# ubc-vision/quadraturefields

Measured on AMD Instinct MI355X. Metric: rays/sec at 800x800 Lego (mesh-quadrature render: ray/mesh intersection + hash-grid/MLP field + compositing), higher is better.
Workload: dtype f32

## Files before the change

### quadraturefields_amd/csrc/exact.hip

```cpp
#include "qf_common.h"
#include "bvh.h"

#pragma clang fp contract(off)

namespace {

constexpr int kMaxHits = QF_BVH_MAX_HITS;

__device__ __forceinline__ bool mt_hit(const float4 a, const float4 b, const float4 c, const float ox, const float oy,
                                       const float oz, const float dx, const float dy, const float dz, float *t_out)
{
    const float e1x = b.x - a.x, e1y = b.y - a.y, e1z = b.z - a.z;
    const float e2x = c.x - a.x, e2y = c.y - a.y, e2z = c.z - a.z;
    const float px = dy * e2z - dz * e2y;
    const float py = dz * e2x - dx * e2z;
    const float pz = dx * e2y - dy * e2x;
    const float det = (e1x * px + e1y * py) + e1z * pz;
    if (!(det != 0.0f)) return false;
    const float inv = 1.0f / det;
    const float tx = ox - a.x, ty = oy - a.y, tz = oz - a.z;
    const float u = ((tx * px + ty * py) + tz * pz) * inv;
    if (!(u >= 0.0f && u <= 1.0f)) return false;
    const float qx = ty * e1z - tz * e1y;
    const float qy = tz * e1x - tx * e1z;
    const float qz = tx * e1y - ty * e1x;
    const float v = ((dx * qx + dy * qy) + dz * qz) * inv;
    if (!(v >= 0.0f && u + v <= 1.0f)) return false;
    const float t = ((e2x * qx + e2y * qy) + e2z * qz) * inv;
    if (!(t > 0.0f)) return false;
    *t_out = t;
    return true;
}

__device__ __forceinline__ float safe_inv(float d)
{
    const float tiny = 1e-30f;
    if (fabsf(d) < tiny) d = (d < 0.0f || (d == 0.0f && signbit(d))) ? -tiny : tiny;
    return 1.0f / d;
}

__device__ __forceinline__ bool hit_less(float ta, int ia, float tb, int ib) { return ta < tb || (ta == tb && ia < ib); }

typedef float f32x4u __attribute__((ext_vector_type(4), aligned(4)));
typedef int i32x4u __attribute__((ext_vector_type(4), aligned(4)));

__device__ __forceinline__ uint64_t hit_key(float t, int id) { return ((uint64_t)__float_as_uint(t) << 32) | (uint32_t)id; }
__device__ __forceinline__ float key_t(uint64_t k) { return __uint_as_float((uint32_t)(k >> 32)); }
__device__ __forceinline__ int key_id(uint64_t k) { return (int)(uint32_t)k; }

template <bool kTri>
__device__ __forceinline__ void sort_row_32(float *row_t, int32_t *row_i, int cnt)
{
    if (kTri) {
        uint64_t key[32];
#pragma unroll
        for (int k = 0; k < 32; ++k) key[k] = k < cnt ? hit_key(row_t[k], row_i[k]) : ~0ull;
#pragma unroll
        for (int k = 2; k <= 32; k <<= 1) {
#pragma unroll
            for (int i = 0; i < 32; ++i) {
                const int l = i ^ (k - 1);
                if (l > i) { const uint64_t a = key[i], b = key[l]; key[i] = a < b ? a : b; key[l] = a < b ? b : a; }
            }
#pragma unroll
            for (int j = k >> 2; j > 0; j >>= 1) {
#pragma unroll
                for (int i = 0; i < 32; ++i) {
                    const int l = i ^ j;
                    if (l > i) { const uint64_t a = key[i], b = key[l]; key[i] = a < b ? a : b; key[l] = a < b ? b : a; }
                }
            }
        }
#pragma unroll
        for (int k = 0; k < 32; ++k)
            if (k < cnt) { row_t[k] = key_t(key[k]); row_i[k] = key_id(key[k]); }
    } else {
        float key[32];
#pragma unroll
        for (int k = 0; k < 32; ++k) key[k] = k < cnt ? row_t[k] : INFINITY;
#pragma unroll
        for (int k = 2; k <= 32; k <<= 1) {
#pragma unroll
            for (int i = 0; i < 32; ++i) {
                const int l = i ^ (k - 1);
                if (l > i) { const float a = key[i], b = key[l]; key[i] = fminf(a, b); key[l] = fmaxf(a, b); }
            }
#pragma unroll
            for (int j = k >> 2; j > 0; j >>= 1) {
#pragma unroll
                for (int i = 0; i < 32; ++i) {
                    const int l = i ^ j;
                    if (l > i) { const float a = key[i], b = key[l]; key[i] = fminf(a, b); key[l] = fmaxf(a, b); }
                }
            }
        }
#pragma unroll
        for (int k = 0; k < 32; ++k)
            if (k < cnt) row_t[k] = key[k];
    }
}

constexpr int kOctRays = 32;
constexpr int kTravThreads = kOctRays * 8;
constexpr int kDone = (int)0x80000000;
constexpr int kMaxPages = 4096;

#define QF_DPP_QUAD_1032 0xB1
#define QF_DPP_QUAD_2301 0x4E
#define QF_DPP_HALF_MIRROR 0x141

__device__ __forceinline__ unsigned oct_min_u32(unsigned v)
{
    v = min(v, (unsigned)__builtin_amdgcn_update_dpp(0, (int)v, QF_DPP_QUAD_1032, 0xf, 0xf, true));
    v = min(v, (unsigned)__builtin_amdgcn_update_dpp(0, (int)v, QF_DPP_QUAD_2301, 0xf, 0xf, true));
    v = min(v, (unsigned)__builtin_amdgcn_update_dpp(0, (int)v, QF_DPP_HALF_MIRROR, 0xf, 0xf, true));
    return v;
}
__device__ __forceinline__ unsigned oct_max_u32(unsigned v)
{
    v = max(v, (unsigned)__builtin_amdgcn_update_dpp(0, (int)v, QF_DPP_QUAD_1032, 0xf, 0xf, true));
    v = max(v, (unsigned)__builtin_amdgcn_update_dpp(0, (int)v, QF_DPP_QUAD_2301, 0xf, 0xf, true));
    v = max(v, (unsigned)__builtin_amdgcn_update_dpp(0, (int)v, QF_DPP_HALF_MIRROR, 0xf, 0xf, true));
    return v;
}
template <int kCtrl>
__device__ __forceinline__ uint64_t dpp_u64(uint64_t v)
{
    const unsigned lo = (unsigned)__builtin_amdgcn_update_dpp(0, (int)(unsigned)v, kCtrl, 0xf, 0xf, true);
    const unsigned hi = (unsigned)__builtin_amdgcn_update_dpp(0, (int)(unsigned)(v >> 32), kCtrl, 0xf, 0xf, true);
    return ((uint64_t)hi << 32) | lo;
}
__device__ __forceinline__ uint64_t oct_max_u64(uint64_t v)
{
    uint64_t o = dpp_u64<QF_DPP_QUAD_1032>(v); v = o > v ? o : v;
    o = dpp_u64<QF_DPP_QUAD_2301>(v); v = o > v ? o : v;
    o = dpp_u64<QF_DPP_HALF_MIRROR>(v); v = o > v ? o : v;
    return v;
}
__device__ __forceinline__ int oct_bcast(int v, int oct_base, int src)
{
    return __builtin_amdgcn_ds_bpermute((oct_base + src) << 2, v);
}
__device__ __forceinline__ void oct_lds_sync()
{
    __builtin_amdgcn_fence(__ATOMIC_ACQ_REL, "wavefront");
    __builtin_amdgcn_wave_barrier();
}

struct OctList {
    uint64_t *keys;
    int K, j;
    int count;
    uint64_t worst;
    int worst_slot;

    __device__ __forceinline__ void find_worst()
    {
        uint64_t m = 0;
        int slot = 0;
        for (int i = j; i < K; i += 8) {
            const uint64_t k = keys[i];
            if (k >= m) { m = k; slot = i; }
        }
        worst = oct_max_u64(m);
        worst_slot = (int)oct_max_u32(m == worst ? (unsigned)slot : 0u);
    }
};

struct TravArgs {
    const float4 *nodes, *tris;
    const float *rays_o, *rays_d;
    int64_t n_rays;
    int root_is_valid, max_hits, image_width, image_height, tiles_x, n_blocks, blocks_per_xcd, stack_cap;
    int stripe_blocks;
    int list_cap;
    float min_sep;
    int32_t *hit_tri;
    float *hit_t;
    int32_t *hit_count;
    uint64_t *keep_mask;
    int32_t *raw_count;
    int tcol_offset;
    const int32_t *all_flag;
};

extern __shared__ uint64_t trav_lds[];

__device__ __forceinline__ uint64_t oct_keep_mask(const TravArgs &a, int64_t ray, int c, int j, int q, int *kept_out)
{
    const int K = a.max_hits, Kc = a.list_cap;
    uint64_t *keys = trav_lds + (size_t)q * Kc;
    uint64_t *sorted = trav_lds + (size_t)kOctRays * Kc + (size_t)q * Kc;
    for (int e = j; e < c; e += 8) keys[e] = hit_key(a.hit_t[ray * K + e], a.hit_tri[ray * K + e]);
    oct_lds_sync();
    for (int e = j; e < c; e += 8) {
        const uint64_t k = keys[e];
        int rank = 0;
        for (int i = 0; i < c; ++i) rank += keys[i] < k ? 1 : 0;
        sorted[rank] = k;
    }
    oct_lds_sync();
    float last = key_t(sorted[0]);
    int kept = 1;
    uint64_t mask = 1ull;
    for (int i = 1; i < c; ++i) {
        const float t = key_t(sorted[i]);
        if (t > last + a.min_sep) { mask |= 1ull << i; ++kept; last = t; }
    }
    oct_lds_sync();
    *kept_out = kept;
    return mask;
}

template <bool kOrdered>
__device__ __forceinline__ void oct_traverse_ray(const TravArgs &ta, int64_t ray, int j, int q, int oct_base)
{
    const int K = ta.max_hits;
    const int Kc = ta.list_cap;
    const float min_sep = ta.min_sep;
    const float4 *__restrict__ nodes = ta.nodes;
    const float4 *__restrict__ tris = ta.tris;
    const int stack_cap = ta.stack_cap;
    uint64_t *keys = trav_lds + (size_t)q * Kc;
    uint64_t *sorted = trav_lds + (size_t)kOctRays * Kc + (size_t)q * Kc;
    int *stack = reinterpret_cast<int *>(trav_lds + (size_t)kOctRays * Kc * (min_sep > 0.0f ? 2 : 1)) + (size_t)q * stack_cap;
    const float *rays_o = ta.rays_o, *rays_d = ta.rays_d;
    const int root_is_valid = ta.root_is_valid;
    float *hit_t = ta.hit_t;
    int32_t *hit_tri = ta.hit_tri, *hit_count = ta.hit_count;
    uint64_t *keep_mask = ta.keep_mask;
    int32_t *raw_count = ta.raw_count;
    const float ox = rays_o[ray * 3], oy = rays_o[ray * 3 + 1], oz = rays_o[ray * 3 + 2];
    const float dx = rays_d[ray * 3], dy = rays_d[ray * 3 + 1], dz = rays_d[ray * 3 + 2];
    const float ix = safe_inv(dx), iy = safe_inv(dy), iz = safe_inv(dz);
    const float nx = -(ox * ix), ny = -(oy * iy), nz = -(oz * iz);
    float *my_t = hit_t + ray * K;
    int32_t *my_tri = hit_tri + ray * K;

    OctList list;
    list.keys = keys; list.K = Kc; list.j = j;
    int kept = 0;
    float last_t = 0.0f;
    uint64_t lo_key = 0;
    float t_lo = 0.0f, t_accept = 0.0f;

    for (int page = 0; page < kMaxPages; ++page) {
        list.count = 0;
        list.worst = ~0ull;
        list.worst_slot = 0;
        float t_limit = INFINITY;
        int sp = 0;
        int cur = root_is_valid ? 0 : kDone;
        while (cur != kDone) {
            while (cur >= 0) {
                const float4 *np = nodes + (size_t)cur * 16 + j * 2;
                const float4 a = np[0];
                const float4 b = np[1];
                const float ax = __builtin_fmaf(a.x, ix, nx), bx = __builtin_fmaf(a.w, ix, nx);
                const float ay = __builtin_fmaf(a.y, iy, ny), by = __builtin_fmaf(b.x, iy, ny);
                const float az = __builtin_fmaf(a.z, iz, nz), bz = __builtin_fmaf(b.y, iz, nz);
                const float tn = fmaxf(fmaxf(fminf(ax, bx), fminf(ay, by)), fmaxf(fminf(az, bz), 0.0f));
                const float tf = fminf(fminf(fmaxf(ax, bx), fmaxf(ay, by)), fmaxf(az, bz)) * 1.0000005f;
                const int tok = __float_as_int(b.z);
                const bool hit = tok != kDone && !(tn > tf) && !(tn * 0.999999f > t_limit) && !(tf < t_lo);
                const unsigned m8 = (unsigned)(__ballot(hit) >> oct_base) & 0xffu;
                if (m8 == 0) {
                    cur = kDone;
                    if (sp > 0) cur = stack[--sp];
                    continue;
                }
                const int n = __popc(m8);
                int nearest;
                if (kOrdered) {
                    const unsigned key = hit ? ((__float_as_uint(tn) & ~7u) | (unsigned)j) : 0xffffffffu;
                    nearest = (int)(oct_min_u32(key) & 7u);
                } else {
                    nearest = __ffs(m8) - 1;
                }
                if (hit && j != nearest) {
                    const unsigned others = m8 & ~(1u << nearest);
                    stack[sp + __popc(others & ((1u << j) - 1u))] = tok;
                }
                sp += n - 1;
                cur = oct_bcast(tok, oct_base, nearest);
                oct_lds_sync();
            }
            if (cur == kDone) break;
            {
                const int packed = ~cur;
                const int first = packed >> 3, cnt = (packed & 7) + 1;
                bool h = false;
                uint64_t key = 0;
                if (j < cnt) {
                    const float4 a = tris[(size_t)(first + j) * 3 + 0];
                    const float4 b = tris[(size_t)(first + j) * 3 + 1];
                    const float4 c = tris[(size_t)(first + j) * 3 + 2];
                    float t;
                    if (mt_hit(a, b, c, ox, oy, oz, dx, dy, dz, &t)) {
                        key = hit_key(t, __float_as_int(a.w));
                        h = key > lo_key && t > t_accept && key < list.worst;
                    }
                }
                const unsigned m8 = (unsigned)(__ballot(h) >> oct_base) & 0xffu;
                if (m8) {
                    const int n = __popc(m8);
                    if (list.count + n <= Kc) {
                        if (h) keys[list.count + __popc(m8 & ((1u << j) - 1u))] = key;
                        list.count += n;
                        oct_lds_sync();
                        if (list.count == Kc) list.find_worst();
                    } else {
                        for (unsigned mm = m8; mm; mm &= mm - 1u) {
                            const int src = __ffs(mm) - 1;
                            const uint64_t k = ((uint64_t)(unsigned)oct_bcast((int)(unsigned)(key >> 32), oct_base, src) << 32) |
                                               (unsigned)oct_bcast((int)(unsigned)key, oct_base, src);
                            if (list.count < Kc) {
                                if (j == 0) keys[list.count] = k;
                                ++list.count;
                                oct_lds_sync();
                                if (list.count == Kc) list.find_worst();
                            } else if (k < list.worst) {
                                if (j == 0) keys[list.worst_slot] = k;
                                oct_lds_sync();
                                list.find_worst();
                            }
                        }
                    }
                    if (list.count == Kc) t_limit = key_t(list.worst);
                }
            }
            cur = kDone;
            if (sp > 0) cur = stack[--sp];
        }

        const int count = list.count;
        if (!(min_sep > 0.0f)) {
            for (int e = j; e < count; e += 8) {
                const uint64_t k = keys[e];
                int rank = 0;
                for (int i = 0; i < count; ++i) rank += keys[i] < k ? 1 : 0;
                my_t[rank] = key_t(k);
                my_tri[rank] = key_id(k);
            }
            kept = count;
            break;
        }
        for (int e = j; e < count; e += 8) {
            const uint64_t k = keys[e];
            int rank = 0;
            for (int i = 0; i < count; ++i) rank += keys[i] < k ? 1 : 0;
            sorted[rank] = k;
        }
        oct_lds_sync();
        for (int i = 0; i < count && kept < K; ++i) {
            const uint64_t k = sorted[i];
            const float t = key_t(k);
            if (kept == 0 || t > last_t + min_sep) {
                if (j == 0) { my_t[kept] = t; my_tri[kept] = key_id(k); }
                ++kept;
                last_t = t;
            }
        }
        if (count < Kc || kept >= K) break;
        lo_key = sorted[Kc - 1];
        t_lo = key_t(lo_key) * 0.999999f;
        t_accept = last_t + min_sep;
        oct_lds_sync();
    }
    for (int i = kept + j; i < K; i += 8) { my_t[i] = INFINITY; my_tri[i] = -1; }
    if (j == 0) {
        hit_count[ray] = kept;
        if (keep_mask) { keep_mask[ray] = kept >= 64 ? ~0ull : ((1ull << kept) - 1ull); raw_count[ray] = kept; }
    }
}

__device__ __forceinline__ int xcd_block(const TravArgs &a)
{
    const int x = (int)(blockIdx.x & 7), k = (int)(blockIdx.x >> 3);
    if (a.stripe_blocks > 0) {
        const int s = k / a.stripe_blocks, p = k - s * a.stripe_blocks;
        return (s * 8 + x) * a.stripe_blocks + p;
    }
    return x * a.blocks_per_xcd + k;
}

template <bool kOrdered>
__global__ __launch_bounds__(kTravThreads) void bvh8_traverse_kernel(TravArgs a)
{
    const int tid = threadIdx.x, j = tid & 7, q = tid >> 3;
    const int oct_base = (tid & 63) & 56;
    const int block = xcd_block(a);
    if (block >= a.n_blocks) return;
    int64_t ray;
    if (a.image_width > 0) {
        const int w = q >> 3, r = q & 7;
        const int px = (block % a.tiles_x) * 8 + (w & 1) * 4 + (r & 3);
        const int py = (block / a.tiles_x) * 4 + (w >> 1) * 2 + (r >> 2);
        if (px >= a.image_width || py >= a.image_height) return;
        ray = (int64_t)py * a.image_width + px;
    } else {
        ray = (int64_t)block * kOctRays + q;
    }
    if (ray >= a.n_rays) return;
    oct_traverse_ray<kOrdered>(a, ray, j, q, oct_base);
}

__global__ __launch_bounds__(kTravThreads) void bvh8_repair_kernel(TravArgs a)
{
    __shared__ int s_list[kTravThreads];
    __shared__ int s_n;
    const int tid = threadIdx.x, j = tid & 7, q = tid >> 3;
    const int oct_base = (tid & 63) & 56;
    const int block = (int)blockIdx.x;
    if (block >= a.n_blocks) return;
    const int K = a.max_hits;
    if (tid == 0) s_n = 0;
    __syncthreads();
    const int64_t ray0 = (int64_t)block * kTravThreads;
    {
        const int64_t ray = ray0 + tid;
        if (ray < a.n_rays) {
            const int c = a.hit_count[ray];
            int need = 0;
            if (c > K || (a.all_flag && *a.all_flag)) need = 2;
            else if (a.keep_mask) {
                bool close_pair = false;
                if (c >= 2) {
                    const float *row = a.hit_t + ray * K;
                    float *col = reinterpret_cast<float *>(trav_lds) + a.tcol_offset + tid;
                    for (int i0 = 0; i0 < c; i0 += 8) {
                        float v[8];
#pragma unroll
                        for (int u = 0; u < 8; ++u) v[u] = (i0 + u < c) ? row[i0 + u] : 0.0f;
#pragma unroll
                        for (int u = 0; u < 8; ++u)
                            if (i0 + u < c) col[(i0 + u) * kTravThreads] = v[u];
                    }
                    const float ms = a.min_sep * 1.0001f;
                    for (int i = 1; i < c; ++i) {
                        const float ti = col[i * kTravThreads];
                        for (int k = 0; k < i; ++k) {
                            const float tk = col[k * kTravThreads];
                            close_pair |= !(fabsf(ti - tk) > ms + 4e-7f * fmaxf(ti, tk));
                        }
                    }
                }
                if (close_pair) need = 1;
                else { a.keep_mask[ray] = c >= 64 ? ~0ull : ((1ull << c) - 1ull); a.raw_count[ray] = c; }
            }
            if (need) s_list[atomicAdd(&s_n, 1)] = tid | (need << 16);
        }
    }
    __syncthreads();
    const int n = s_n;
    for (int e = q; e < n; e += kOctRays) {
        const int entry = s_list[e];
        const int64_t ray = ray0 + (entry & 0xffff);
        if ((entry >> 16) == 2) {
            oct_traverse_ray<true>(a, ray, j, q, oct_base);
        } else {
            const int c = a.hit_count[ray];
            int kept;
            const uint64_t mask = oct_keep_mask(a, ray, c, j, q, &kept);
            if (j == 0) { a.keep_mask[ray] = mask; a.raw_count[ray] = c; a.hit_count[ray] = kept; }
        }
    }
}

struct RasterCam {
    float r00, r01, r02, r10, r11, r12, r20, r21, r22;
    float cx, cy, cz;
    float fx, fy, px0, py0;
    int w, h;
};

constexpr float kRasterGuard = 0.25f;

struct SlabArgs {
    float t_lo, t_hi;
    int stop_at;
    uint64_t *keys;
    const float4 *ray_rec;
};

struct TriSetup {
    int x0, x1, y0, y1;
    bool use_edges;
    float ea[3], eb[3], ec[3];
};

__device__ __forceinline__ bool tri_setup(const float4 a, const float4 b, const float4 c, const RasterCam &cam, TriSetup &s)
{
    float minx = INFINITY, maxx = -INFINITY, miny = INFINITY, maxy = -INFINITY;
    int behind = 0;
    const float4 vs[3] = {a, b, c};
    float sxs[3], sys[3];
#pragma unroll
    for (int k = 0; k < 3; ++k) {
        const float dx = vs[k].x - cam.cx, dy = vs[k].y - cam.cy, dz = vs[k].z - cam.cz;
        const float xc = cam.r00 * dx + cam.r10 * dy + cam.r20 * dz;
        const float yc = cam.r01 * dx + cam.r11 * dy + cam.r21 * dz;
        const float zc = cam.r02 * dx + cam.r12 * dy + cam.r22 * dz;
        const float zv = -zc;
        if (!(zv > 1e-6f)) { ++behind; sxs[k] = sys[k] = 0.0f; continue; }
        const float sx = cam.fx * (xc / zv) + cam.px0;
        const float sy = -cam.fy * (yc / zv) + cam.py0;
        sxs[k] = sx; sys[k] = sy;
        minx = fminf(minx, sx); maxx = fmaxf(maxx, sx);
        miny = fminf(miny, sy); maxy = fmaxf(maxy, sy);
    }
    if (behind == 3) return false;
    s.use_edges = false;
    if (behind > 0) {
        s.x0 = 0; s.y0 = 0; s.x1 = cam.w - 1; s.y1 = cam.h - 1;
    } else {
        s.x0 = (int)fmaxf(floorf(minx - kRasterGuard), 0.0f);
        s.y0 = (int)fmaxf(floorf(miny - kRasterGuard), 0.0f);
        s.x1 = (int)fminf(ceilf(maxx + kRasterGuard), (float)(cam.w - 1));
        s.y1 = (int)fminf(ceilf(maxy + kRasterGuard), (float)(cam.h - 1));
        if (!(maxx + kRasterGuard >= 0.0f) || !(maxy + kRasterGuard >= 0.0f) ||
            !(minx - kRasterGuard <= (float)(cam.w - 1)) || !(miny - kRasterGuard <= (float)(cam.h - 1)))
            return false;
        const float area2 = (sxs[1] - sxs[0]) * (sys[2] - sys[0]) - (sys[1] - sys[0]) * (sxs[2] - sxs[0]);
        if (fabsf(area2) > 1e-2f) {
            s.use_edges = true;
            const float sgn = area2 > 0.0f ? 1.0f : -1.0f;
#pragma unroll
            for (int k = 0; k < 3; ++k) {
                const int k1 = (k + 1) % 3;
                const float ex = sxs[k1] - sxs[k], ey = sys[k1] - sys[k];
                s.ea[k] = -sgn * ey;
                s.eb[k] = sgn * ex;
                s.ec[k] = -(s.ea[k] * sxs[k] + s.eb[k] * sys[k]) + (kRasterGuard + 0.05f) * (fabsf(ex) + fabsf(ey)) + 1e-3f;
            }
        }
    }
    return true;
}

template <int kRasterLanes, bool kWide, bool kSlab = false>
__device__ __forceinline__ void raster_triangle(const float4 *__restrict__ tris, int64_t tri_i, int sub, const RasterCam &cam,
                                                const float *__restrict__ rays_o, const float *__restrict__ rays_d,
                                                int max_hits, int32_t *__restrict__ hit_tri, float *__restrict__ hit_t,
                                                int32_t *__restrict__ hit_count, int32_t *__restrict__ overflow,
                                                const bool cam_origin, const SlabArgs slab = SlabArgs())
{
    const float4 a = tris[tri_i * 3 + 0], b = tris[tri_i * 3 + 1], c = tris[tri_i * 3 + 2];
    const int id = __float_as_int(a.w);
    TriSetup ts;
    if (!tri_setup(a, b, c, cam, ts)) return;
    const int x0 = ts.x0, x1 = ts.x1, y0 = ts.y0, y1 = ts.y1;
    const bool use_edges = ts.use_edges;
    const float *ea = ts.ea, *eb = ts.eb, *ec = ts.ec;
    const int bw = x1 - x0 + 1;
    const int total = bw * (y1 - y0 + 1);
    int px = x0 + sub % bw, py = y0 + sub / bw;
    for (int q = sub; q < total; q += kRasterLanes) {
        const int cx_ = px, cy_ = py;
        px += kRasterLanes;
        while (px > x1) { px -= bw; ++py; }
        if (use_edges) {
            const float fx_ = (float)cx_, fy_ = (float)cy_;
            if (ea[0] * fx_ + eb[0] * fy_ + ec[0] < 0.0f || ea[1] * fx_ + eb[1] * fy_ + ec[1] < 0.0f ||
                ea[2] * fx_ + eb[2] * fy_ + ec[2] < 0.0f)
                continue;
        }
        const int64_t ray = (int64_t)cy_ * cam.w + cx_;
        float dx, dy, dz;
        if (kSlab && slab.ray_rec) {
            const float4 rr = slab.ray_rec[ray];
            if (__float_as_int(rr.w) >= slab.stop_at) continue;
            dx = rr.x; dy = rr.y; dz = rr.z;
        } else {
            dx = rays_d[ray * 3]; dy = rays_d[ray * 3 + 1]; dz = rays_d[ray * 3 + 2];
        }
        float ox = cam.cx, oy = cam.cy, oz = cam.cz;
        if (!cam_origin) { ox = rays_o[ray * 3]; oy = rays_o[ray * 3 + 1]; oz = rays_o[ray * 3 + 2]; }
        asm volatile("" : "+v"(ox), "+v"(oy), "+v"(oz), "+v"(dx), "+v"(dy), "+v"(dz));
        float t;
        if (!mt_hit(a, b, c, ox, oy, oz, dx, dy, dz, &t)) continue;
        if (kSlab) {
            if (!(t >= slab.t_lo && t < slab.t_hi)) continue;
            const int slot = atomicAdd(&hit_count[ray], 1);
            if (slot < max_hits) slab.keys[(int64_t)slot * ((int64_t)cam.w * cam.h) + ray] = hit_key(t, id);
            else atomicAdd(overflow, 1);
            continue;
        }
        const int slot = atomicAdd(&hit_count[ray], 1);
        if (slot < max_hits) {
            const int64_t at = kWide ? (int64_t)slot * ((int64_t)cam.w * cam.h) + ray : ray * max_hits + slot;
            hit_t[at] = t;
            if (hit_tri) hit_tri[at] = id;
        } else {
            atomicAdd(overflow, 1);
        }
    }
}

template <int kRasterLanes, bool kWide>
__global__ __launch_bounds__(256) void raster_kernel(const float4 *__restrict__ tris, int64_t n_tri, RasterCam cam,
                                                     const float *__restrict__ rays_o, const float *__restrict__ rays_d,
                                                     int max_hits, int32_t *__restrict__ hit_tri, float *__restrict__ hit_t,
                                                     int32_t *__restrict__ hit_count, int32_t *__restrict__ overflow,
                                                     const int32_t *__restrict__ ray_flag)
{
    const int64_t gid = (int64_t)blockIdx.x * blockDim.x + threadIdx.x;
    const int64_t tri_i = gid / kRasterLanes;
    const int sub = (int)(gid % kRasterLanes);
    if (tri_i >= n_tri) return;
    if (ray_flag && *ray_flag) return;
    const bool cam_origin = ray_flag != nullptr;
    raster_triangle<kRasterLanes, kWide>(tris, tri_i, sub, cam, rays_o, rays_d, max_hits, hit_tri, hit_t, hit_count, overflow,
                                         cam_origin);
}

constexpr float kRayPixelTol = 0.02f;
constexpr float kRayUnitTol = 1e-4f;

__device__ __forceinline__ void camera_rays_check(const uint32_t *__restrict__ o_bits, const float *__restrict__ rays_d,
                                                  int64_t n_rays, const RasterCam &cam, int32_t *__restrict__ flag,
                                                  int64_t first, int64_t stride)
{
    const uint32_t c0 = __float_as_uint(cam.cx), c1 = __float_as_uint(cam.cy), c2 = __float_as_uint(cam.cz);
    bool bad = false;
    for (int64_t r = first; r < n_rays; r += stride) {
        const uint32_t o0 = o_bits[r * 3], o1 = o_bits[r * 3 + 1], o2 = o_bits[r * 3 + 2];
        const float dx = rays_d[r * 3], dy = rays_d[r * 3 + 1], dz = rays_d[r * 3 + 2];
        bad = bad || o0 != c0 || o1 != c1 || o2 != c2;
        const float xc = cam.r00 * dx + cam.r10 * dy + cam.r20 * dz;
        const float yc = cam.r01 * dx + cam.r11 * dy + cam.r21 * dz;
        const float zv = -(cam.r02 * dx + cam.r12 * dy + cam.r22 * dz);
        const float sx = cam.fx * (xc / zv) + cam.px0, sy = -cam.fy * (yc / zv) + cam.py0;
        const float px = (float)(int)(r % cam.w), py = (float)(int)(r / cam.w);
        bad = bad || !(zv > 0.0f) || !(fabsf(sx - px) <= kRayPixelTol) || !(fabsf(sy - py) <= kRayPixelTol) ||
              !(fabsf(dx * dx + dy * dy + dz * dz - 1.0f) <= kRayUnitTol);
    }
    if (bad) *flag = 1;
}

__global__ void camera_rays_check_kernel(const uint32_t *__restrict__ o_bits, const float *__restrict__ rays_d, int64_t n_rays,
                                         RasterCam cam, int32_t *__restrict__ flag)
{
    camera_rays_check(o_bits, rays_d, n_rays, cam, flag, (int64_t)blockIdx.x * blockDim.x + threadIdx.x,
                      (int64_t)gridDim.x * blockDim.x);
}

constexpr int kCullChunk = 64;

__global__ __launch_bounds__(256) void chunk_boxes_kernel(const float4 *__restrict__ tris, int64_t n_tri, int n_chunks,
                                                          float4 *__restrict__ boxes)
{
    const int chunk = (int)(((int64_t)blockIdx.x * blockDim.x + threadIdx.x) >> 6), lane = threadIdx.x & 63;
    if (chunk >= n_chunks) return;
    const int64_t t = (int64_t)chunk * kCullChunk + lane;
    float lo[3] = {INFINITY, INFINITY, INFINITY}, hi[3] = {-INFINITY, -INFINITY, -INFINITY};
    if (t < n_tri) {
#pragma unroll
        for (int k = 0; k < 3; ++k) {
            const float4 v = tris[t * 3 + k];
            lo[0] = fminf(lo[0], v.x); lo[1] = fminf(lo[1], v.y); lo[2] = fminf(lo[2], v.z);
            hi[0] = fmaxf(hi[0], v.x); hi[1] = fmaxf(hi[1], v.y); hi[2] = fmaxf(hi[2], v.z);
        }
    }
#pragma unroll
    for (int off = 32; off > 0; off >>= 1) {
#pragma unroll
        for (int k = 0; k < 3; ++k) {
            lo[k] = fminf(lo[k], __shfl_xor(lo[k], off, 64));
            hi[k] = fmaxf(hi[k], __shfl_xor(hi[k], off, 64));
        }
    }
    if (lane == 0) {
        boxes[chunk * 2 + 0] = make_float4(lo[0], lo[1], lo[2], 0.0f);
        boxes[chunk * 2 + 1] = make_float4(hi[0], hi[1], hi[2], 0.0f);
    }
}

__global__ void cull_chunks_kernel(const float4 *__restrict__ boxes, int n_chunks, RasterCam cam, int32_t *__restrict__ visible,
                                   int32_t *__restrict__ counters, int parity, const uint32_t *__restrict__ o_bits,
                                   const float *__restrict__ rays_d, int64_t n_rays, int32_t *__restrict__ ray_flag)
{
    const int chunk = blockIdx.x * blockDim.x + threadIdx.x;
    if (chunk == 0) counters[parity ^ 1] = 0;
    if (ray_flag) camera_rays_check(o_bits, rays_d, n_rays, cam, ray_flag, chunk, (int64_t)gridDim.x * blockDim.x);
    if (chunk >= n_chunks) return;
    const float4 lo = boxes[chunk * 2], hi = boxes[chunk * 2 + 1];
    if (!(lo.x <= hi.x)) return;
    float minx = INFINITY, maxx = -INFINITY, miny = INFINITY, maxy = -INFINITY;
    bool keep = false;
#pragma unroll
    for (int k = 0; k < 8; ++k) {
        const float dx = ((k & 1) ? hi.x : lo.x) - cam.cx, dy = ((k & 2) ? hi.y : lo.y) - cam.cy, dz = ((k & 4) ? hi.z : lo.z) - cam.cz;
        const float xc = cam.r00 * dx + cam.r10 * dy + cam.r20 * dz;
        const float yc = cam.r01 * dx + cam.r11 * dy + cam.r21 * dz;
        const float zc = cam.r02 * dx + cam.r12 * dy + cam.r22 * dz;
        const float zv = -zc;
        if (!(zv > 1e-4f)) { keep = true; continue; }
        const float sx = cam.fx * (xc / zv) + cam.px0, sy = -cam.fy * (yc / zv) + cam.py0;
        minx = fminf(minx, sx); maxx = fmaxf(maxx, sx);
        miny = fminf(miny, sy); maxy = fmaxf(maxy, sy);
    }
    const float g = kRasterGuard + 1.0f;
    if (!keep)
        keep = (maxx + g >= 0.0f) && (maxy + g >= 0.0f) && (minx - g <= (float)(cam.w - 1)) && (miny - g <= (float)(cam.h - 1));
    if (keep) visible[atomicAdd(&counters[parity], 1)] = chunk;
}

template <int kRasterLanes, bool kWide>
__global__ __launch_bounds__(256) void raster_culled_kernel(const float4 *__restrict__ tris, int64_t n_tri, RasterCam cam,
                                                            const float *__restrict__ rays_o, const float *__restrict__ rays_d,
                                                            int max_hits, int32_t *__restrict__ hit_tri, float *__restrict__ hit_t,
                                                            int32_t *__restrict__ hit_count, int32_t *__restrict__ overflow,
                                                            const int32_t *__restrict__ visible, const int32_t *__restrict__ n_visible,
                                                            const int32_t *__restrict__ ray_flag)
{
    if (ray_flag && *ray_flag) return;
    const bool cam_origin = ray_flag != nullptr;
    constexpr int kTrisPerBlock = 256 / kRasterLanes;
    constexpr int kBlocksPerChunk = kCullChunk / kTrisPerBlock;
    const int n_items = *n_visible * kBlocksPerChunk;
    const int sub = threadIdx.x % kRasterLanes;
    for (int item = blockIdx.x; item < n_items; item += gridDim.x) {
        const int chunk = visible[item / kBlocksPerChunk];
        const int64_t tri_i = (int64_t)chunk * kCullChunk + (item % kBlocksPerChunk) * kTrisPerBlock + threadIdx.x / kRasterLanes;
        if (tri_i < n_tri)
            raster_triangle<kRasterLanes, kWide>(tris, tri_i, sub, cam, rays_o, rays_d, max_hits, hit_tri, hit_t, hit_count, overflow,
                                                 cam_origin);
    }
}

constexpr int kMaxSlabs = 16;

struct SlabCtl {
    uint32_t dist_min_bits, dist_max_bits;
    int32_t n_visible;
    int32_t slab_count[kMaxSlabs];
};

__device__ __forceinline__ void slab_range(const SlabCtl *ctl, int n_slabs, float *lo, float *width)
{
    const float dmin = __uint_as_float(ctl->dist_min_bits) * 0.999f, dmax = __uint_as_float(ctl->dist_max_bits) * 1.001f;
    *lo = dmin;
    *width = fmaxf(dmax - dmin, 1e-12f) / (float)n_slabs;
}

__device__ __forceinline__ void slab_edges(const SlabCtl *ctl, int n_slabs, int j, float *t_lo, float *t_hi)
{
#pragma clang fp contract(off)
    float lo, w;
    slab_range(ctl, n_slabs, &lo, &w);
    *t_lo = j == 0 ? -INFINITY : lo + (float)j * w;
    *t_hi = j == n_slabs - 1 ? INFINITY : lo + (float)(j + 1) * w;
}

__global__ void slab_cull_kernel(const float4 *__restrict__ boxes, int n_chunks, RasterCam cam, int32_t *__restrict__ visible,
                                 float2 *__restrict__ range, SlabCtl *ctl)
{
    const int chunk = blockIdx.x * blockDim.x + threadIdx.x;
    if (chunk >= n_chunks) return;
    const float4 lo = boxes[chunk * 2], hi = boxes[chunk * 2 + 1];
    if (!(lo.x <= hi.x)) return;
    float minx = INFINITY, maxx = -INFINITY, miny = INFINITY, maxy = -INFINITY;
    bool keep = false;
#pragma unroll
    for (int k = 0; k < 8; ++k) {
        const float dx = ((k & 1) ? hi.x : lo.x) - cam.cx, dy = ((k & 2) ? hi.y : lo.y) - cam.cy, dz = ((k & 4) ? hi.z : lo.z) - cam.cz;
        const float xc = cam.r00 * dx + cam.r10 * dy + cam.r20 * dz;
        const float yc = cam.r01 * dx + cam.r11 * dy + cam.r21 * dz;
        const float zc = cam.r02 * dx + cam.r12 * dy + cam.r22 * dz;
        const float zv = -zc;
        if (!(zv > 1e-4f)) { keep = true; continue; }
        const float sx = cam.fx * (xc / zv) + cam.px0, sy = -cam.fy * (yc / zv) + cam.py0;
        minx = fminf(minx, sx); maxx = fmaxf(maxx, sx);
        miny = fminf(miny, sy); maxy = fmaxf(maxy, sy);
    }
    const float g = kRasterGuard + 1.0f;
    if (!keep)
        keep = (maxx + g >= 0.0f) && (maxy + g >= 0.0f) && (minx - g <= (float)(cam.w - 1)) && (miny - g <= (float)(cam.h - 1));
    if (!keep) return;
    const float nx = fmaxf(fmaxf(lo.x - cam.cx, cam.cx - hi.x), 0.0f), ny = fmaxf(fmaxf(lo.y - cam.cy, cam.cy - hi.y), 0.0f);
    const float nz = fmaxf(fmaxf(lo.z - cam.cz, cam.cz - hi.z), 0.0f);
    const float fx = fmaxf(fabsf(lo.x - cam.cx), fabsf(hi.x - cam.cx)), fy = fmaxf(fabsf(lo.y - cam.cy), fabsf(hi.y - cam.cy));
    const float fz = fmaxf(fabsf(lo.z - cam.cz), fabsf(hi.z - cam.cz));
    const float dmin = sqrtf(nx * nx + ny * ny + nz * nz) * 0.9999f, dmax = sqrtf(fx * fx + fy * fy + fz * fz) * 1.0001f + 1e-30f;
    visible[atomicAdd(&ctl->n_visible, 1)] = chunk;
    range[chunk] = make_float2(dmin, dmax);
    atomicMin(&ctl->dist_min_bits, __float_as_uint(dmin));
    atomicMax(&ctl->dist_max_bits, __float_as_uint(dmax));
}

__global__ __launch_bounds__(256) void slab_assign_kernel(const int32_t *__restrict__ visible, const float2 *__restrict__ range,
                                                          SlabCtl *ctl, int n_slabs, int n_chunks, int32_t *__restrict__ lists)
{
    __shared__ int s_cnt[kMaxSlabs], s_base[kMaxSlabs];
    if (threadIdx.x < kMaxSlabs) s_cnt[threadIdx.x] = 0;
    __syncthreads();
    const int e = blockIdx.x * blockDim.x + threadIdx.x;
    int chunk = -1, j0 = 0, j1 = -1;
    if (e < ctl->n_visible) {
        chunk = visible[e];
        const float2 r = range[chunk];
        const float dlo = r.x * 0.999f, dhi = r.y * 1.001f;
        j0 = n_slabs;
        for (int j = 0; j < n_slabs; ++j) {
            float t_lo, t_hi;
            slab_edges(ctl, n_slabs, j, &t_lo, &t_hi);
            if (t_hi > dlo && t_lo <= dhi) { j0 = j < j0 ? j : j0; j1 = j; }
        }
        for (int j = j0; j <= j1; ++j) atomicAdd(&s_cnt[j], 1);
    }
    __syncthreads();
    if (threadIdx.x < n_slabs) s_base[threadIdx.x] = s_cnt[threadIdx.x] ? atomicAdd(&ctl->slab_count[threadIdx.x], s_cnt[threadIdx.x]) : 0;
    __syncthreads();
    for (int j = j0; j <= j1; ++j) lists[(int64_t)j * n_chunks + atomicAdd(&s_base[j], 1)] = chunk;
}

__global__ void slab_ray_records_kernel(const float *__restrict__ rays_d, const int32_t *__restrict__ hit_count, int64_t n,
                                        float4 *__restrict__ rec)
{
    for (int64_t i = (int64_t)blockIdx.x * blockDim.x + threadIdx.x; i < n; i += (int64_t)gridDim.x * blockDim.x)
        rec[i] = make_float4(rays_d[i * 3], rays_d[i * 3 + 1], rays_d[i * 3 + 2], __int_as_float(hit_count[i]));
}

template <int kRasterLanes>
__global__ __launch_bounds__(256) void raster_slab_kernel(const float4 *__restrict__ tris, int64_t n_tri, RasterCam cam,
                                                          const float *__restrict__ rays_o, const float *__restrict__ rays_d,
                                                          int capacity, uint64_t *__restrict__ keys, int32_t *__restrict__ hit_count,
                                                          int32_t *__restrict__ overflow, const int32_t *__restrict__ list,
                                                          const SlabCtl *__restrict__ ctl, int slab_j, int n_slabs, int stop_at,
                                                          const float4 *__restrict__ ray_rec,
                                                          const int32_t *__restrict__ ray_flag)
{
    if (ray_flag && *ray_flag) return;
    const bool cam_origin = ray_flag != nullptr;
    constexpr int kTrisPerBlock = 256 / kRasterLanes;
    constexpr int kBlocksPerChunk = kCullChunk / kTrisPerBlock;
    const int n_items = ctl->slab_count[slab_j] * kBlocksPerChunk;
    SlabArgs sa;
    slab_edges(ctl, n_slabs, slab_j, &sa.t_lo, &sa.t_hi);
    sa.stop_at = stop_at;
    sa.keys = keys;
    sa.ray_rec = ray_rec;
    const int sub = threadIdx.x % kRasterLanes;
    for (int item = blockIdx.x; item < n_items; item += gridDim.x) {
        const int chunk = list[item / kBlocksPerChunk];
        const int64_t tri_i = (int64_t)chunk * kCullChunk + (item % kBlocksPerChunk) * kTrisPerBlock + threadIdx.x / kRasterLanes;
        if (tri_i < n_tri)
            raster_triangle<kRasterLanes, true, true>(tris, tri_i, sub, cam, rays_o, rays_d, capacity, nullptr, nullptr,
                                                      hit_count, overflow, cam_origin, sa);
    }
}

constexpr int kSelectBlock = 64;
constexpr int kSelectHeadroom = 8;
__host__ __device__ inline int select_capacity(int max_hits, int wide, float min_sep)
{
    const int cap = min_sep > 0.0f ? max_hits + kSelectHeadroom : max_hits;
    return cap < wide ? cap : wide;
}
__device__ __forceinline__ void write_row_from_keys(const uint64_t *lk, int count, float *row_t, int32_t *row_i)
{
    int i = 0;
    for (; i + 4 <= count; i += 4) {
        f32x4u t4;
        i32x4u i4;
#pragma unroll
        for (int e = 0; e < 4; ++e) {
            const uint64_t k = lk[(i + e) * kSelectBlock];
            t4[e] = key_t(k);
            i4[e] = key_id(k);
        }
        *reinterpret_cast<f32x4u *>(row_t + i) = t4;
        *reinterpret_cast<i32x4u *>(row_i + i) = i4;
    }
    for (; i < count; ++i) {
        const uint64_t k = lk[i * kSelectBlock];
        row_t[i] = key_t(k);
        row_i[i] = key_id(k);
    }
}

template <bool kKeys>
__global__ __launch_bounds__(kSelectBlock) void select_nearest_kernel(int64_t n_rays, int wide, int max_hits, float min_sep,
                                                                      const int32_t *__restrict__ wide_tri,
                                                                      const float *__restrict__ wide_t,
                                                                      const uint64_t *__restrict__ wide_key,
                                                                      int32_t *__restrict__ hit_tri, float *__restrict__ hit_t,
                                                                      int32_t *__restrict__ hit_count)
{
    extern __shared__ __attribute__((aligned(8))) unsigned char select_lds[];
    const int cap = select_capacity(max_hits, wide, min_sep);
    uint64_t *lk = reinterpret_cast<uint64_t *>(select_lds) + threadIdx.x;
    const int64_t r = (int64_t)blockIdx.x * kSelectBlock + threadIdx.x;
    if (r >= n_rays) return;
    const int cnt = hit_count[r];
    if (cnt > wide) return;
    float *row_t = hit_t + r * max_hits;
    int32_t *row_i = hit_tri + r * max_hits;
    if (cnt <= max_hits) {
        constexpr int kCopy = 8;
        for (int i0 = 0; i0 < cnt; i0 += kCopy) {
            float tb[kCopy];
            int ib[kCopy];
#pragma unroll
            for (int u = 0; u < kCopy; ++u) {
                const int i = i0 + u < cnt ? i0 + u : cnt - 1;
                if (kKeys) {
                    const uint64_t k = wide_key[(int64_t)i * n_rays + r];
                    tb[u] = key_t(k);
                    ib[u] = key_id(k);
                } else {
                    tb[u] = wide_t[(int64_t)i * n_rays + r];
                    ib[u] = wide_tri[(int64_t)i * n_rays + r];
                }
            }
#pragma unroll
            for (int q = 0; q < kCopy / 4; ++q) {
                if (i0 + 4 * q + 4 <= cnt) {
                    *reinterpret_cast<f32x4u *>(row_t + i0 + 4 * q) = (f32x4u){tb[4 * q], tb[4 * q + 1], tb[4 * q + 2], tb[4 * q + 3]};
                    *reinterpret_cast<i32x4u *>(row_i + i0 + 4 * q) = (i32x4u){ib[4 * q], ib[4 * q + 1], ib[4 * q + 2], ib[4 * q + 3]};
                } else {
#pragma unroll
                    for (int e = 0; e < 4; ++e)
                        if (i0 + 4 * q + e < cnt) { row_t[i0 + 4 * q + e] = tb[4 * q + e]; row_i[i0 + 4 * q + e] = ib[4 * q + e]; }
                }
            }
        }
        return;
    }
    const int held = cnt < cap ? cnt : cap;
    constexpr int kBatch = 8;
    int n = 0;
    uint64_t max_key = 0;
    for (int i0 = 0; i0 < cnt; i0 += kBatch) {
        uint64_t kb[kBatch];
#pragma unroll
        for (int u = 0; u < kBatch; ++u) {
            const int i = i0 + u < cnt ? i0 + u : cnt - 1;
            if (kKeys) kb[u] = wide_key[(int64_t)i * n_rays + r];
            else kb[u] = hit_key(wide_t[(int64_t)i * n_rays + r], wide_tri[(int64_t)i * n_rays + r]);
        }
#pragma unroll
        for (int u = 0; u < kBatch; ++u) {
            if (i0 + u >= cnt) break;
            const uint64_t key = kb[u];
            int m;
            if (n < held) {
                m = n;
                ++n;
            } else {
                if (!(key < max_key)) continue;
                m = n - 1;
            }
            int lo = 0, hi = m;
            while (lo < hi) {
                const int mid = (lo + hi) >> 1;
                if (lk[mid * kSelectBlock] < key) lo = mid + 1;
                else hi = mid;
            }
            int j = m - 1;
            for (; j - 3 >= lo; j -= 4) {
                const uint64_t a0 = lk[j * kSelectBlock], a1 = lk[(j - 1) * kSelectBlock], a2 = lk[(j - 2) * kSelectBlock],
                               a3 = lk[(j - 3) * kSelectBlock];
                lk[(j + 1) * kSelectBlock] = a0;
                lk[j * kSelectBlock] = a1;
                lk[(j - 1) * kSelectBlock] = a2;
                lk[(j - 2) * kSelectBlock] = a3;
            }
            for (; j >= lo; --j) lk[(j + 1) * kSelectBlock] = lk[j * kSelectBlock];
            lk[lo * kSelectBlock] = key;
            max_key = lk[(n - 1) * kSelectBlock];
        }
    }
    if (min_sep <= 0.0f) {
        write_row_from_keys(lk, max_hits, row_t, row_i);
        hit_count[r] = max_hits;
        return;
    }
    float last_t = key_t(lk[0]);
    int kept = 1;
    for (int i = 1; i < held && kept < max_hits; ++i) {
        const uint64_t k = lk[i * kSelectBlock];
        const float t = key_t(k);
        if (!(t > last_t + min_sep)) continue;
        last_t = t;
        lk[kept * kSelectBlock] = k;
        ++kept;
    }
    if (kept < max_hits && cnt > held) return;
    write_row_from_keys(lk, kept, row_t, row_i);
    hit_count[r] = kept;
}

constexpr int kFilterRays = 128;
__global__ __launch_bounds__(kFilterRays) void filter_hits_kernel(int64_t n_rays, int max_hits, float min_sep,
                                                                  int32_t *__restrict__ hit_tri, float *__restrict__ hit_t,
                                                                  int32_t *__restrict__ hit_count)
{
    extern __shared__ __attribute__((aligned(16))) unsigned char filter_smem[];
    const int K = max_hits, Kp = max_hits | 1;
    float *s_t = reinterpret_cast<float *>(filter_smem);
    int32_t *s_tri = reinterpret_cast<int32_t *>(s_t + kFilterRays * Kp);
    const int tid = threadIdx.x;
    const int64_t ray0 = (int64_t)blockIdx.x * kFilterRays;
    const int nr = (int)((n_rays - ray0) < kFilterRays ? (n_rays - ray0) : kFilterRays);
    for (int i = tid; i < nr * K; i += kFilterRays) {
        const int r = i / K, k = i - r * K;
        s_t[r * Kp + k] = hit_t[ray0 * K + i];
        s_tri[r * Kp + k] = hit_tri[ray0 * K + i];
    }
    __syncthreads();
    if (tid < nr) {
        int cnt = hit_count[ray0 + tid];
        if (cnt > K) cnt = K;
        float *row_t = s_t + tid * Kp;
        int32_t *row_i = s_tri + tid * Kp;
        if (K <= 32) {
            if (cnt > 1) sort_row_32<true>(row_t, row_i, cnt);
        } else {
            for (int i = 1; i < cnt; ++i) {
                const float t = row_t[i];
                const int id = row_i[i];
                int j = i - 1;
                while (j >= 0 && hit_less(t, id, row_t[j], row_i[j])) { row_t[j + 1] = row_t[j]; row_i[j + 1] = row_i[j]; --j; }
                row_t[j + 1] = t;
                row_i[j + 1] = id;
            }
        }
        if (min_sep > 0.0f && cnt > 1) {
            int kept = 1;
            float last_t = row_t[0];
            for (int i = 1; i < cnt; ++i) {
                const float t = row_t[i];
                if (t > last_t + min_sep) { row_t[kept] = t; row_i[kept] = row_i[i]; ++kept; last_t = t; }
            }
            cnt = kept;
        }
        for (int i = cnt; i < K; ++i) { row_t[i] = INFINITY; row_i[i] = -1; }
        hit_count[ray0 + tid] = cnt;
    }
    __syncthreads();
    for (int i = tid; i < nr * K; i += kFilterRays) {
        const int r = i / K, k = i - r * K;
        hit_t[ray0 * K + i] = s_t[r * Kp + k];
        hit_tri[ray0 * K + i] = s_tri[r * Kp + k];
    }
}

template <int kN, bool kTri>
__device__ __forceinline__ void load_sort_row(const float *__restrict__ g_t, const int32_t *__restrict__ g_i, int K,
                                              int cnt, int deepest, float *row_t, int32_t *row_i)
{
    float t[kN];
    int32_t id[kN];
#pragma unroll
    for (int j = 0; j < kN / 4; ++j) {
        f32x4u v = {INFINITY, INFINITY, INFINITY, INFINITY};
        i32x4u w = {-1, -1, -1, -1};
        if (4 * j < deepest) {
            if (4 * j + 3 < K) {
                v = *reinterpret_cast<const f32x4u *>(g_t + 4 * j);
                if (kTri) w = *reinterpret_cast<const i32x4u *>(g_i + 4 * j);
            } else {
#pragma unroll
                for (int e = 0; e < 3; ++e)
                    if (4 * j + e < K) {
                        v[e] = g_t[4 * j + e];
                        if (kTri) w[e] = g_i[4 * j + e];
                    }
            }
        }
#pragma unroll
        for (int e = 0; e < 4; ++e) { t[4 * j + e] = v[e]; id[4 * j + e] = w[e]; }
    }
    if (kTri) {
        uint64_t key[kN];
#pragma unroll
        for (int k = 0; k < kN; ++k) key[k] = k < cnt ? hit_key(t[k], id[k]) : ~0ull;
#pragma unroll
        for (int k = 2; k <= kN; k <<= 1) {
#pragma unroll
            for (int i = 0; i < kN; ++i) {
                const int l = i ^ (k - 1);
                if (l > i) { const uint64_t a = key[i], b = key[l]; key[i] = a < b ? a : b; key[l] = a < b ? b : a; }
            }
#pragma unroll
            for (int j = k >> 2; j > 0; j >>= 1) {
#pragma unroll
                for (int i = 0; i < kN; ++i) {
                    const int l = i ^ j;
                    if (l > i) { const uint64_t a = key[i], b = key[l]; key[i] = a < b ? a : b; key[l] = a < b ? b : a; }
                }
            }
        }
#pragma unroll
        for (int k = 0; k < kN; ++k)
            if (k < cnt) { row_t[k] = key_t(key[k]); row_i[k] = key_id(key[k]); }
    } else {
#pragma unroll
        for (int k = 0; k < kN; ++k) t[k] = k < cnt ? t[k] : INFINITY;
#pragma unroll
        for (int k = 2; k <= kN; k <<= 1) {
#pragma unroll
            for (int i = 0; i < kN; ++i) {
                const int l = i ^ (k - 1);
                if (l > i) { const float a = t[i], b = t[l]; t[i] = fminf(a, b); t[l] = fmaxf(a, b); }
            }
#pragma unroll
            for (int j = k >> 2; j > 0; j >>= 1) {
#pragma unroll
                for (int i = 0; i < kN; ++i) {
                    const int l = i ^ j;
                    if (l > i) { const float a = t[i], b = t[l]; t[i] = fminf(a, b); t[l] = fmaxf(a, b); }
                }
            }
        }
#pragma unroll
        for (int k = 0; k < kN; ++k)
            if (k < cnt) row_t[k] = t[k];
    }
}

constexpr int kPackRays = 128;

__device__ __forceinline__ double sample_depth64(float t, const double o[3], const double d[3], double p[3])
{
    const double td = (double)t;
    p[0] = o[0] + td * d[0];
    p[1] = o[1] + td * d[1];
    p[2] = o[2] + td * d[2];
    const double qx = p[0] - o[0], qy = p[1] - o[1], qz = p[2] - o[2];
    return sqrt((qx * qx + qy * qy) + qz * qz);
}

__global__ __launch_bounds__(kPackRays) void pack_samples_kernel(
    const float *__restrict__ rays_o, const float *__restrict__ rays_d, int64_t n_rays, int max_hits,
    const int32_t *__restrict__ hit_tri, const float *__restrict__ hit_t, const int32_t *__restrict__ hit_count,
    const int64_t *__restrict__ ray_offset, float *__restrict__ xyz, float *__restrict__ dirs,
    int64_t *__restrict__ index_ray, float *__restrict__ depth, int64_t *__restrict__ index_tri,
    float *__restrict__ origins, const int32_t *__restrict__ inverse, float *__restrict__ xyz_c,
    float *__restrict__ dirs_c, float *__restrict__ depth_c, const uint64_t *__restrict__ keep_mask,
    const int32_t *__restrict__ raw_count, float min_sep, int32_t *__restrict__ close_flag)
{
    extern __shared__ __attribute__((aligned(16))) unsigned char smem[];
    const int K = max_hits, Kp = max_hits | 1;
    float *s_t = reinterpret_cast<float *>(smem);
    int32_t *s_tri = reinterpret_cast<int32_t *>(s_t + kPackRays * Kp);
    uint16_t *s_map = reinterpret_cast<uint16_t *>(s_tri + kPackRays * Kp);
    __shared__ int s_region;

    const int tid = threadIdx.x;
    const int64_t ray0 = (int64_t)blockIdx.x * kPackRays;
    const int nr = (int)((n_rays - ray0) < kPackRays ? (n_rays - ray0) : kPackRays);
    int cnt = 0;
    if (tid < nr) {
        cnt = keep_mask ? raw_count[ray0 + tid] : hit_count[ray0 + tid];
        if (cnt > K) cnt = K;
    }
    if (K <= 32) {
        int deepest = cnt;
#pragma unroll
        for (int off = 32; off > 0; off >>= 1) {
            const int other = __shfl_xor(deepest, off, 64);
            deepest = other > deepest ? other : deepest;
        }
        const int64_t own = tid < nr ? ray0 + tid : ray0;
        if (deepest > 16) load_sort_row<32, true>(hit_t + own * K, hit_tri + own * K, K, cnt, deepest, s_t + tid * Kp, s_tri + tid * Kp);
        else if (deepest > 0) load_sort_row<16, true>(hit_t + own * K, hit_tri + own * K, K, cnt, deepest, s_t + tid * Kp, s_tri + tid * Kp);
    } else {
        for (int i = tid; i < nr * K; i += kPackRays) {
            const int r = i / K, k = i - r * K;
            s_t[r * Kp + k] = hit_t[ray0 * K + i];
            s_tri[r * Kp + k] = hit_tri[ray0 * K + i];
        }
    }
    if (tid == 0) s_region = 0;
    __syncthreads();

    const int64_t block_base = ray_offset[ray0];
    if (tid < nr) {
        const int64_t ray = ray0 + tid;
        float *row_t = s_t + tid * Kp;
        int32_t *row_i = s_tri + tid * Kp;
        if (K > 32) {
            for (int i = 1; i < cnt; ++i) {
                const float t = row_t[i];
                const int id = row_i[i];
                int j = i - 1;
                while (j >= 0 && hit_less(t, id, row_t[j], row_i[j])) { row_t[j + 1] = row_t[j]; row_i[j + 1] = row_i[j]; --j; }
                row_t[j + 1] = t;
                row_i[j + 1] = id;
            }
        }
        if (keep_mask) {
            const uint64_t mask = keep_mask[ray];
            int kept = 0;
            for (int i = 0; i < cnt; ++i)
                if ((mask >> i) & 1ull) { row_t[kept] = row_t[i]; row_i[kept] = row_i[i]; ++kept; }
            cnt = kept;
        } else if (close_flag && min_sep > 0.0f) {
            bool drop = false;
            for (int i = 1; i < cnt; ++i) drop |= !(row_t[i] > row_t[i - 1] + min_sep);
            if (drop) *close_flag = 1;
        }
        if (cnt > 1) {
            const double o64[3] = {(double)rays_o[ray * 3], (double)rays_o[ray * 3 + 1], (double)rays_o[ray * 3 + 2]};
            const double d64[3] = {(double)rays_d[ray * 3], (double)rays_d[ray * 3 + 1], (double)rays_d[ray * 3 + 2]};
            double p[3];
            double prev = sample_depth64(row_t[0], o64, d64, p);
            bool sorted = true;
            for (int k = 1; k < cnt; ++k) {
                const double dk = sample_depth64(row_t[k], o64, d64, p);
                sorted = sorted && !(prev > dk);
                prev = dk;
            }
            if (!sorted) {
                for (int i = 1; i < cnt; ++i) {
                    const float t = row_t[i];
                    const int id = row_i[i];
                    const double di = sample_depth64(t, o64, d64, p);
                    int j = i - 1;
                    while (j >= 0 && sample_depth64(row_t[j], o64, d64, p) > di) { row_t[j + 1] = row_t[j]; row_i[j + 1] = row_i[j]; --j; }
                    row_t[j + 1] = t;
                    row_i[j + 1] = id;
                }
            }
        }
        const int local = (int)(ray_offset[ray] - block_base);
        for (int k = 0; k < cnt; ++k) s_map[local + k] = (uint16_t)((tid << 8) | k);
        if (tid == nr - 1) s_region = local + cnt;
    }
    __syncthreads();

    const int region = s_region;
    for (int j = tid; j < region; j += kPackRays) {
        const int m = s_map[j];
        const int rl = m >> 8, k = m & 255;
        const int64_t ray = ray0 + rl;
        const float ox = rays_o[ray * 3], oy = rays_o[ray * 3 + 1], oz = rays_o[ray * 3 + 2];
        const float dx = rays_d[ray * 3], dy = rays_d[ray * 3 + 1], dz = rays_d[ray * 3 + 2];
        const double o64[3] = {(double)ox, (double)oy, (double)oz};
        const double d64[3] = {(double)dx, (double)dy, (double)dz};
        double p[3];
        const double dep = sample_depth64(s_t[rl * Kp + k], o64, d64, p);
        const float nrm = sqrtf((dx * dx + dy * dy) + dz * dz) + 1e-7f;
        const int64_t o = block_base + j;
        if (xyz) {
            xyz[o * 3 + 0] = (float)p[0];
            xyz[o * 3 + 1] = (float)p[1];
            xyz[o * 3 + 2] = (float)p[2];
            dirs[o * 3 + 0] = dx / nrm;
            dirs[o * 3 + 1] = dy / nrm;
            dirs[o * 3 + 2] = dz / nrm;
            origins[o * 3 + 0] = ox;
            origins[o * 3 + 1] = oy;
            origins[o * 3 + 2] = oz;
        }
        index_ray[o] = ray;
        depth[o] = (float)dep;
        index_tri[o] = (int64_t)s_tri[rl * Kp + k];
        if (inverse) {
            const int64_t c = inverse[o];
            xyz_c[c * 3 + 0] = (float)p[0];
            xyz_c[c * 3 + 1] = (float)p[1];
            xyz_c[c * 3 + 2] = (float)p[2];
            dirs_c[c * 3 + 0] = dx / nrm;
            dirs_c[c * 3 + 1] = dy / nrm;
            dirs_c[c * 3 + 2] = dz / nrm;
            if (depth_c) depth_c[c] = (float)dep;
        }
    }
}

template <bool kTri>
__global__ __launch_bounds__(64) void pack_tiles_kernel(
    const float *__restrict__ rays_o, const float *__restrict__ rays_d, int w, int h, int tiles_x, int n_tiles, int max_hits,
    const int32_t *__restrict__ hit_tri, const float *__restrict__ hit_t, const int32_t *__restrict__ hit_count,
    const int64_t *__restrict__ tile_base, const int64_t *__restrict__ total, float *__restrict__ xyz_c,
    float *__restrict__ dirs_c, float *__restrict__ depth_c, int32_t *__restrict__ tri_c, const uint64_t *__restrict__ keep_mask,
    const int32_t *__restrict__ raw_count, float min_sep, int32_t *__restrict__ final_count, int32_t *__restrict__ dropped)
{
    extern __shared__ __attribute__((aligned(16))) unsigned char smem[];
    const int K = max_hits, Kp = max_hits | 1;
    float *s_t = reinterpret_cast<float *>(smem);
    int32_t *s_tri = reinterpret_cast<int32_t *>(s_t + 64 * Kp);
    const int tile = blockIdx.x, lane = threadIdx.x;
    const int px0 = (tile % tiles_x) * 8, py0 = (tile / tiles_x) * 8;
    const int cols = (w - px0) < 8 ? (w - px0) : 8, rows = (h - py0) < 8 ? (h - py0) : 8;
    const int px = px0 + (lane & 7), py = py0 + (lane >> 3);
    const bool inside = px < w && py < h;
    const int64_t ray = inside ? (int64_t)py * w + px : 0;
    int cnt = 0;
    if (inside) {
        cnt = keep_mask ? raw_count[ray] : hit_count[ray];
        if (cnt > K) cnt = K;
    }
    int deepest = cnt;
#pragma unroll
    for (int off = 32; off > 0; off >>= 1) {
        const int other = __shfl_xor(deepest, off, 64);
        deepest = other > deepest ? other : deepest;
    }
    if (deepest == 0) {
        if (final_count && inside) final_count[ray] = 0;
        return;
    }
    float *row_t = s_t + lane * Kp;
    int32_t *row_i = s_tri + lane * Kp;
    const float ox = rays_o[ray * 3], oy = rays_o[ray * 3 + 1], oz = rays_o[ray * 3 + 2];
    const float dx = rays_d[ray * 3], dy = rays_d[ray * 3 + 1], dz = rays_d[ray * 3 + 2];
    int64_t base = tile_base[tile];
    if (K <= 32) {
        if (deepest <= 16) load_sort_row<16, kTri>(hit_t + ray * K, hit_tri + ray * K, K, cnt, deepest, row_t, row_i);
        else load_sort_row<32, kTri>(hit_t + ray * K, hit_tri + ray * K, K, cnt, deepest, row_t, row_i);
    } else {
        for (int yy = 0; yy < rows; ++yy) {
            const int64_t row_ray0 = (int64_t)(py0 + yy) * w + px0;
            for (int i = lane; i < cols * deepest; i += 64) {
                const int r = i / deepest, k = i - r * deepest;
                s_t[(yy * 8 + r) * Kp + k] = hit_t[(row_ray0 + r) * K + k];
                if (kTri) s_tri[(yy * 8 + r) * Kp + k] = hit_tri[(row_ray0 + r) * K + k];
            }
        }
        __syncthreads();
    }
    double o64[3] = {0.0, 0.0, 0.0}, d64[3] = {0.0, 0.0, 0.0};
    float dn[3] = {0.0f, 0.0f, 0.0f};
    int n_dropped = 0;
    if (inside) {
        if (K > 32) {
            for (int i = 1; i < cnt; ++i) {
                const float t = row_t[i];
                const int id = kTri ? row_i[i] : 0;
                int j = i - 1;
                while (j >= 0 && (kTri ? hit_less(t, id, row_t[j], row_i[j]) : t < row_t[j])) {
                    row_t[j + 1] = row_t[j];
                    if (kTri) row_i[j + 1] = row_i[j];
                    --j;
                }
                row_t[j + 1] = t;
                if (kTri) row_i[j + 1] = id;
            }
        }
        if (keep_mask) {
            const uint64_t mask = keep_mask[ray];
            int kept = 0;
            for (int i = 0; i < cnt; ++i)
                if ((mask >> i) & 1ull) { row_t[kept] = row_t[i]; if (kTri) row_i[kept] = row_i[i]; ++kept; }
            cnt = kept;
        } else if (min_sep > 0.0f && cnt > 1) {
            float last_t = row_t[0];
            int kept = 1;
            for (int i = 1; i < cnt; ++i) {
                const float t = row_t[i];
                if (t > last_t + min_sep) { row_t[kept] = t; if (kTri) row_i[kept] = row_i[i]; ++kept; last_t = t; }
            }
            n_dropped = cnt - kept;
            cnt = kept;
        }
        if (cnt > 0) {
            o64[0] = (double)ox; o64[1] = (double)oy; o64[2] = (double)oz;
            d64[0] = (double)dx; d64[1] = (double)dy; d64[2] = (double)dz;
            const float nrm = sqrtf((dx * dx + dy * dy) + dz * dz) + 1e-7f;
            dn[0] = dx / nrm; dn[1] = dy / nrm; dn[2] = dz / nrm;
        }
        if (cnt > 1) {
            double p[3];
            double prev = sample_depth64(row_t[0], o64, d64, p);
            bool sorted = true;
            for (int k = 1; k < cnt; ++k) {
                const double dk = sample_depth64(row_t[k], o64, d64, p);
                sorted = sorted && !(prev > dk);
                prev = dk;
            }
            if (!sorted) {
                for (int i = 1; i < cnt; ++i) {
                    const float t = row_t[i];
                    const int id = kTri ? row_i[i] : 0;
                    const double di = sample_depth64(t, o64, d64, p);
                    int j = i - 1;
                    while (j >= 0 && sample_depth64(row_t[j], o64, d64, p) > di) {
                        row_t[j + 1] = row_t[j];
                        if (kTri) row_i[j + 1] = row_i[j];
                        --j;
                    }
                    row_t[j + 1] = t;
                    if (kTri) row_i[j + 1] = id;
                }
            }
        }
    }
    if (final_count && inside) final_count[ray] = cnt;
    const unsigned long long below = (1ull << lane) - 1ull;
    float first_xyz[3] = {0.0f, 0.0f, 0.0f};
    for (int k = 0;; ++k) {
        const unsigned long long mask = __ballot(cnt > k);
        if (mask == 0ull) break;
        if (cnt > k) {
            const int64_t c = base + __popcll(mask & below);
            double p[3];
            const double dep = sample_depth64(row_t[k], o64, d64, p);
            xyz_c[c * 3 + 0] = (float)p[0];
            xyz_c[c * 3 + 1] = (float)p[1];
            xyz_c[c * 3 + 2] = (float)p[2];
            dirs_c[c * 3 + 0] = dn[0];
            dirs_c[c * 3 + 1] = dn[1];
            dirs_c[c * 3 + 2] = dn[2];
            depth_c[c] = (float)dep;
            if (kTri) tri_c[c] = (int32_t)row_i[k];
            if (k == 0) { first_xyz[0] = (float)p[0]; first_xyz[1] = (float)p[1]; first_xyz[2] = (float)p[2]; }
        }
        base += __popcll(mask);
    }
    const unsigned long long any_drop = __ballot(n_dropped > 0);
    if (any_drop) {
        const int64_t end = tile + 1 < n_tiles ? tile_base[tile + 1] : *total;
        const int src = __ffsll((long long)__ballot(cnt > 0)) - 1;
        const float gx = __shfl(first_xyz[0], src, 64), gy = __shfl(first_xyz[1], src, 64), gz = __shfl(first_xyz[2], src, 64);
        const float hx = __shfl(dn[0], src, 64), hy = __shfl(dn[1], src, 64), hz = __shfl(dn[2], src, 64);
        const int gtri = kTri ? __shfl((int)row_i[0], src, 64) : 0;
        for (int64_t c = base + lane; c < end; c += 64) {
            xyz_c[c * 3 + 0] = gx; xyz_c[c * 3 + 1] = gy; xyz_c[c * 3 + 2] = gz;
            dirs_c[c * 3 + 0] = hx; dirs_c[c * 3 + 1] = hy; dirs_c[c * 3 + 2] = hz;
            depth_c[c] = 0.0f;
            if (kTri) tri_c[c] = (int32_t)gtri;
        }
        int sum = n_dropped;
#pragma unroll
        for (int off = 32; off > 0; off >>= 1) sum += __shfl_xor(sum, off, 64);
        if (lane == 0 && dropped) atomicAdd(dropped, sum);
    }
}

__global__ void publish_dropped_kernel(int32_t *dropped, int64_t *host_out)
{
    host_out[2] = (int64_t)*dropped;
    *dropped = 0;
}

__global__ void resort_kernel(const int64_t *index_ray, const float *depth, int64_t n, int64_t *perm)
{
    for (int64_t i = (int64_t)blockIdx.x * blockDim.x + threadIdx.x; i < n; i += (int64_t)gridDim.x * blockDim.x) {
        const int64_t ray = index_ray[i];
        if (i != 0 && index_ray[i - 1] == ray) continue;
        perm[i] = i;
        for (int64_t k = i + 1; k < n && index_ray[k] == ray; ++k) {
            const float dk = depth[k];
            int64_t j = k - 1;
            while (j >= i && depth[perm[j]] > dk) { perm[j + 1] = perm[j]; --j; }
            perm[j + 1] = k;
        }
    }
}

constexpr int RS_THREADS = 256;
constexpr int RS_CHUNK = 1024;
constexpr int RS_HALO = 64;
constexpr int RS_STAGE = RS_CHUNK + RS_HALO;

__global__ __launch_bounds__(RS_THREADS) void resort_samples_kernel(
    const int64_t *index_ray, const float *depth, int64_t n, const float *points, const float *origins,
    const float *vectors, const int64_t *index_tri, int64_t *perm, float *out_points, float *out_depth,
    float *out_origins, float *out_vectors, int64_t *out_index_tri, uint8_t *boundary, const int32_t *inverse,
    float *out_points_c, float *out_vectors_c)
{
    __shared__ float s_depth[RS_STAGE];
    __shared__ int64_t s_ray[RS_STAGE + 1];
    __shared__ int s_src[RS_STAGE];
    __shared__ uint8_t s_mine[RS_STAGE];
    __shared__ int s_heads[RS_CHUNK];
    __shared__ int s_nheads;
    const int64_t n_chunks = (n + RS_CHUNK - 1) / RS_CHUNK;
    for (int64_t chunk = blockIdx.x; chunk < n_chunks; chunk += gridDim.x) {
        const int64_t b0 = chunk * RS_CHUNK;
        const int staged = (int)((n - b0 < RS_STAGE) ? (n - b0) : RS_STAGE);
        const int own = (int)((n - b0 < RS_CHUNK) ? (n - b0) : RS_CHUNK);
        if (threadIdx.x == 0) {
            s_ray[0] = b0 > 0 ? index_ray[b0 - 1] : 0;
            s_nheads = 0;
        }
        for (int k = threadIdx.x; k < staged; k += RS_THREADS) {
            s_depth[k] = depth[b0 + k];
            s_ray[k + 1] = index_ray[b0 + k];
            s_mine[k] = 0;
        }
        __syncthreads();
        for (int k = threadIdx.x; k < own; k += RS_THREADS) {
            const bool head = (b0 + k == 0) || s_ray[k] != s_ray[k + 1];
            if (boundary) boundary[b0 + k] = head ? 1 : 0;
            if (head) s_heads[atomicAdd(&s_nheads, 1)] = k;
        }
        __syncthreads();
        const int n_heads = s_nheads;
        for (int h = threadIdx.x; h < n_heads; h += RS_THREADS) {
            const int k = s_heads[h];
            const int64_t ray = s_ray[k + 1];
            int end = k + 1;
            while (end < staged && s_ray[end + 1] == ray) ++end;
            const bool spills = end == staged && b0 + staged < n && index_ray[b0 + staged] == ray;
            if (!spills) {
                s_src[k] = k;
                s_mine[k] = 1;
                for (int q = k + 1; q < end; ++q) {
                    const float dq = s_depth[q];
                    int j = q - 1;
                    while (j >= k && s_depth[s_src[j]] > dq) { s_src[j + 1] = s_src[j]; --j; }
                    s_src[j + 1] = q;
                    s_mine[q] = 1;
                }
            } else {
                const int64_t i = b0 + k;
                int64_t e = i + 1;
                while (e < n && index_ray[e] == ray) ++e;
                for (int64_t q = i; q < e; ++q) {
                    const float dq = depth[q];
                    int64_t rank = 0;
                    for (int64_t r = i; r < e; ++r) {
                        const float dr = depth[r];
                        rank += (dr < dq) || (dr == dq && r < q);
                    }
                    const int64_t dst = i + rank;
                    if (perm) perm[dst] = q;
                    out_depth[dst] = dq;
                    if (out_index_tri) out_index_tri[dst] = index_tri[q];
                    const int64_t pos_c = inverse ? (int64_t)inverse[dst] : 0;
                    for (int c = 0; c < 3; ++c) {
                        out_points[dst * 3 + c] = points[q * 3 + c];
                        if (out_origins) out_origins[dst * 3 + c] = origins[q * 3 + c];
                        out_vectors[dst * 3 + c] = vectors[q * 3 + c];
                        if (inverse) {
                            out_points_c[pos_c * 3 + c] = points[q * 3 + c];
                            out_vectors_c[pos_c * 3 + c] = vectors[q * 3 + c];
                        }
                    }
                }
            }
        }
        __syncthreads();
        for (int k = threadIdx.x; k < staged; k += RS_THREADS) {
            if (!s_mine[k]) continue;
            const int64_t src = b0 + s_src[k], dst = b0 + k;
            if (perm) perm[dst] = src;
            out_depth[dst] = s_depth[s_src[k]];
            if (out_index_tri) out_index_tri[dst] = index_tri[src];
        }
        for (int e = threadIdx.x; e < 3 * staged; e += RS_THREADS) {
            const int k = e / 3, c = e - 3 * k;
            if (!s_mine[k]) continue;
            const int64_t src = (b0 + s_src[k]) * 3 + c, dst = b0 * 3 + e;
            const float pv = points[src], vv = vectors[src];
            out_points[dst] = pv;
            if (out_origins) out_origins[dst] = origins[src];
            out_vectors[dst] = vv;
            if (inverse) {
                const int64_t pc = (int64_t)inverse[b0 + k] * 3 + c;
                out_points_c[pc] = pv;
                out_vectors_c[pc] = vv;
            }
        }
        __syncthreads();
    }
}

__global__ void texel_indices_kernel(const double *vertices, const int64_t *faces, const float *uv, const float *points,
                                     const int64_t *index_tri, int64_t n, int texture_size, int64_t *texel)
{
    for (int64_t i = (int64_t)blockIdx.x * blockDim.x + threadIdx.x; i < n; i += (int64_t)gridDim.x * blockDim.x) {
        const int64_t f = index_tri[i];
        const int64_t ia = faces[f * 3], ib = faces[f * 3 + 1], ic = faces[f * 3 + 2];
        const double ax = vertices[ia * 3], ay = vertices[ia * 3 + 1], az = vertices[ia * 3 + 2];
        const double e0x = vertices[ib * 3] - ax, e0y = vertices[ib * 3 + 1] - ay, e0z = vertices[ib * 3 + 2] - az;
        const double e1x = vertices[ic * 3] - ax, e1y = vertices[ic * 3 + 1] - ay, e1z = vertices[ic * 3 + 2] - az;
        const double wx = (double)points[i * 3] - ax, wy = (double)points[i * 3 + 1] - ay, wz = (double)points[i * 3 + 2] - az;
        const double d00 = (e0x * e0x + e0y * e0y) + e0z * e0z;
        const double d01 = (e0x * e1x + e0y * e1y) + e0z * e1z;
        const double d11 = (e1x * e1x + e1y * e1y) + e1z * e1z;
        const double d02 = (e0x * wx + e0y * wy) + e0z * wz;
        const double d12 = (e1x * wx + e1y * wy) + e1z * wz;
        const double inv = 1.0 / (d00 * d11 - d01 * d01);
        const double b2d = (d00 * d12 - d01 * d02) * inv;
        const double b1d = (d11 * d02 - d01 * d12) * inv;
        const double b0d = 1.0 - b1d - b2d;
        float b0 = fminf(fmaxf((float)b0d, 0.0f), 1.0f);
        float b1 = fminf(fmaxf((float)b1d, 0.0f), 1.0f);
        float b2 = fminf(fmaxf((float)b2d, 0.0f), 1.0f);
        const float s = (b0 + b1) + b2;
        b0 = b0 / s;
        b1 = b1 / s;
        b2 = b2 / s;
#pragma unroll
        for (int k = 0; k < 2; ++k) {
            const float u = (uv[ia * 2 + k] * b0 + uv[ib * 2 + k] * b1) + uv[ic * 2 + k] * b2;
            float fl = floorf(u);
            int64_t q = (fl != fl) ? 0 : (fl <= -9.2e18f ? INT64_MIN : (fl >= 9.2e18f ? INT64_MAX : (int64_t)fl));
            if (q < 0) q = 0;
            if (q > texture_size - 1) q = texture_size - 1;
            texel[i * 2 + k] = q;
        }
    }
}

struct TexelRecord {
    double ax, ay, az, e0x, e0y, e0z, e1x, e1y, e1z, d00, d01, d11, inv;
    float uv[6];
};
static_assert(sizeof(TexelRecord) == 128, "one 128-byte line per triangle");

__global__ void texel_records_kernel(const double *vertices, const int64_t *faces, const float *uv, int64_t n_faces,
                                     TexelRecord *records)
{
    for (int64_t f = (int64_t)blockIdx.x * blockDim.x + threadIdx.x; f < n_faces; f += (int64_t)gridDim.x * blockDim.x) {
        const int64_t ia = faces[f * 3], ib = faces[f * 3 + 1], ic = faces[f * 3 + 2];
        TexelRecord r;
        r.ax = vertices[ia * 3]; r.ay = vertices[ia * 3 + 1]; r.az = vertices[ia * 3 + 2];
        r.e0x = vertices[ib * 3] - r.ax; r.e0y = vertices[ib * 3 + 1] - r.ay; r.e0z = vertices[ib * 3 + 2] - r.az;
        r.e1x = vertices[ic * 3] - r.ax; r.e1y = vertices[ic * 3 + 1] - r.ay; r.e1z = vertices[ic * 3 + 2] - r.az;
        r.d00 = (r.e0x * r.e0x + r.e0y * r.e0y) + r.e0z * r.e0z;
        r.d01 = (r.e0x * r.e1x + r.e0y * r.e1y) + r.e0z * r.e1z;
        r.d11 = (r.e1x * r.e1x + r.e1y * r.e1y) + r.e1z * r.e1z;
        r.inv = 1.0 / (r.d00 * r.d11 - r.d01 * r.d01);
        r.uv[0] = uv[ia * 2]; r.uv[1] = uv[ia * 2 + 1];
        r.uv[2] = uv[ib * 2]; r.uv[3] = uv[ib * 2 + 1];
        r.uv[4] = uv[ic * 2]; r.uv[5] = uv[ic * 2 + 1];
        records[f] = r;
    }
}

__device__ __forceinline__ void texel_from_record(const TexelRecord &r, float px, float py, float pz, int texture_size,
                                                  int64_t out[2])
{
    const double wx = (double)px - r.ax, wy = (double)py - r.ay, wz = (double)pz - r.az;
    const double d02 = (r.e0x * wx + r.e0y * wy) + r.e0z * wz;
    const double d12 = (r.e1x * wx + r.e1y * wy) + r.e1z * wz;
    const double b2d = (r.d00 * d12 - r.d01 * d02) * r.inv;
    const double b1d = (r.d11 * d02 - r.d01 * d12) * r.inv;
    const double b0d = 1.0 - b1d - b2d;
    float b0 = fminf(fmaxf((float)b0d, 0.0f), 1.0f);
    float b1 = fminf(fmaxf((float)b1d, 0.0f), 1.0f);
    float b2 = fminf(fmaxf((float)b2d, 0.0f), 1.0f);
    const float s = (b0 + b1) + b2;
    b0 = b0 / s;
    b1 = b1 / s;
    b2 = b2 / s;
#pragma unroll
    for (int k = 0; k < 2; ++k) {
        const float u = (r.uv[k] * b0 + r.uv[2 + k] * b1) + r.uv[4 + k] * b2;
        float fl = floorf(u);
        int64_t q = (fl != fl) ? 0 : (fl <= -9.2e18f ? INT64_MIN : (fl >= 9.2e18f ? INT64_MAX : (int64_t)fl));
        if (q < 0) q = 0;
        if (q > texture_size - 1) q = texture_size - 1;
        out[k] = q;
    }
}

__global__ void texel_indices_packed_kernel(const TexelRecord *__restrict__ records, const float *__restrict__ points,
                                            const int64_t *__restrict__ index_tri, int64_t n, int texture_size,
                                            int64_t *__restrict__ texel)
{
    for (int64_t i = (int64_t)blockIdx.x * blockDim.x + threadIdx.x; i < n; i += (int64_t)gridDim.x * blockDim.x) {
        const TexelRecord r = records[index_tri[i]];
        int64_t q[2];
        texel_from_record(r, points[i * 3], points[i * 3 + 1], points[i * 3 + 2], texture_size, q);
        texel[i * 2 + 0] = q[0];
        texel[i * 2 + 1] = q[1];
    }
}

struct TexArgs {
    const uint8_t *alpha, *diffuse;
    const uint8_t *colors[QF_MAX_LOBES];
    const uint8_t *lam[QF_MAX_LOBES];
    int size, n_lobes, sigmoid_codec;
    float lambda_thres;
};

__device__ __forceinline__ float decode_color(uint8_t c, int sigmoid_codec)
{
    const float v = (float)c / 255.0f;
    if (sigmoid_codec) return logf(fminf(fmaxf(v / (1.0f - v), 1e-8f), 1e37f));
    return v * 2.0f * 12.0f - 12.0f;
}

constexpr int kTexelRecord = QF_TEXEL_RECORD_BYTES;

__device__ __forceinline__ void gather_record(const TexArgs &t, int64_t px, uint8_t *rec)
{
    rec[0] = t.alpha[px];
    rec[1] = t.diffuse[px * 3 + 0];
    rec[2] = t.diffuse[px * 3 + 1];
    rec[3] = t.diffuse[px * 3 + 2];
    for (int l = 0; l < t.n_lobes; ++l) {
        uint8_t *r = rec + 4 + 6 * l;
        r[0] = t.lam[l][px * 3 + 0];
        r[1] = t.lam[l][px * 3 + 1];
        r[2] = t.lam[l][px * 3 + 2];
        r[3] = t.colors[l][px * 3 + 0];
        r[4] = t.colors[l][px * 3 + 1];
        r[5] = t.colors[l][px * 3 + 2];
    }
}

__global__ void texture_pack_kernel(TexArgs t, uint8_t *records)
{
    const int64_t n = (int64_t)t.size * t.size;
    for (int64_t px = (int64_t)blockIdx.x * blockDim.x + threadIdx.x; px < n; px += (int64_t)gridDim.x * blockDim.x) {
        union { uint8_t b[kTexelRecord]; uint4 q[kTexelRecord / 16]; } rec;
#pragma unroll
        for (int k = 0; k < kTexelRecord / 16; ++k) rec.q[k] = make_uint4(0u, 0u, 0u, 0u);
        gather_record(t, px, rec.b);
        uint4 *dst = reinterpret_cast<uint4 *>(records + px * kTexelRecord);
#pragma unroll
        for (int k = 0; k < kTexelRecord / 16; ++k) dst[k] = rec.q[k];
    }
}

__device__ __forceinline__ uint32_t rec_byte(const uint32_t (&w)[kTexelRecord / 4], int idx)
{
    return (w[idx >> 2] >> ((idx & 3) * 8)) & 0xffu;
}

template <bool kLookup, typename TriT>
__global__ __launch_bounds__(256) void texture_shade_packed_kernel(const uint8_t *__restrict__ records, int size, int n_lobes,
                                                                   int sigmoid_codec, float lambda_thres,
                                                                   const int64_t *__restrict__ texel,
                                                                   const float *__restrict__ dirs, int64_t n,
                                                                   float *__restrict__ rgb, float *__restrict__ sigma,
                                                                   const TexelRecord *__restrict__ tri_records,
                                                                   const float *__restrict__ points,
                                                                   const TriT *__restrict__ index_tri,
                                                                   const int64_t *__restrict__ n_dev)
{
    if (n_dev) { const int64_t nd = *n_dev; n = nd < n ? (nd > 0 ? nd : 0) : n; }
    __shared__ float s_sigma[256], s_col[256], s_caz[256], s_saz[256], s_sel[256], s_cel[256], s_lam[256];
    {
        const int c = threadIdx.x;
        const float pi = 3.14159274101257324f;
        const float a = (float)c / 255.0f;
        s_sigma[c] = -logf(fmaxf(1.0f - a, 1e-6f)) / 0.005f;
        s_col[c] = decode_color((uint8_t)c, sigmoid_codec);
        const float az = (float)(uint8_t)(c - 128) / 128.0f * pi;
        const float el = (float)c / 256.0f * pi;
        s_caz[c] = cosf(az);
        s_saz[c] = sinf(az);
        s_sel[c] = sinf(el);
        s_cel[c] = cosf(el);
        s_lam[c] = expf((float)c * lambda_thres / 255.0f - 2.5f);
    }
    __syncthreads();
    const int n16 = (4 + 6 * n_lobes + 15) / 16;
    for (int64_t i = (int64_t)blockIdx.x * blockDim.x + threadIdx.x; i < n; i += (int64_t)gridDim.x * blockDim.x) {
        int64_t px;
        if (kLookup) {
            const TexelRecord tr = tri_records[index_tri[i]];
            int64_t rc[2];
            texel_from_record(tr, points[i * 3], points[i * 3 + 1], points[i * 3 + 2], size, rc);
            px = rc[0] * size + rc[1];
        } else {
            px = texel[i * 2] * size + texel[i * 2 + 1];
        }
        const uint4 *src = reinterpret_cast<const uint4 *>(records + px * kTexelRecord);
        uint32_t w[kTexelRecord / 4];
#pragma unroll
        for (int k = 0; k < kTexelRecord / 16; ++k) {
            uint4 q = make_uint4(0u, 0u, 0u, 0u);
            if (k < n16) q = src[k];
            w[4 * k] = q.x; w[4 * k + 1] = q.y; w[4 * k + 2] = q.z; w[4 * k + 3] = q.w;
        }
        const float dx = dirs[i * 3], dy = dirs[i * 3 + 1], dz = dirs[i * 3 + 2];
        float r = 0.0f, g = 0.0f, b = 0.0f;
#pragma unroll
        for (int l = 0; l < QF_MAX_LOBES; ++l) {
            if (l < n_lobes) {
                const int o = 4 + 6 * l;
                const uint32_t c_lam = rec_byte(w, o), c_az = rec_byte(w, o + 1), c_el = rec_byte(w, o + 2);
                const float se = s_sel[c_el];
                const float x0 = s_caz[c_az] * se, x1 = s_saz[c_az] * se, x2 = s_cel[c_el];
                const float nrm = sqrtf((x0 * x0 + x1 * x1) + x2 * x2);
                const float dotp = ((x0 / nrm) * dx + (x1 / nrm) * dy) + (x2 / nrm) * dz;
                const float e = expf(fabsf(s_lam[c_lam]) * (dotp - 1.0f));
                r += s_col[rec_byte(w, o + 3)] * e;
                g += s_col[rec_byte(w, o + 4)] * e;
                b += s_col[rec_byte(w, o + 5)] * e;
            }
        }
        rgb[i * 3 + 0] = 1.0f / (1.0f + expf(-(s_col[rec_byte(w, 1)] + r)));
        rgb[i * 3 + 1] = 1.0f / (1.0f + expf(-(s_col[rec_byte(w, 2)] + g)));
        rgb[i * 3 + 2] = 1.0f / (1.0f + expf(-(s_col[rec_byte(w, 3)] + b)));
        sigma[i] = s_sigma[rec_byte(w, 0)];
    }
}

__device__ __forceinline__ void decode_lobe(const TexArgs &t, int l, int64_t px, float *o )
{
    const uint8_t lc = t.lam[l][px * 3 + 0], az8 = t.lam[l][px * 3 + 1], el8 = t.lam[l][px * 3 + 2];
    const float pi = 3.14159274101257324f;
    const float az = (float)(uint8_t)(az8 - 128) / 128.0f * pi;
    const float el = (float)el8 / 256.0f * pi;
    const float se = sinf(el);
    o[0] = cosf(az) * se;
    o[1] = sinf(az) * se;
    o[2] = cosf(el);
    o[3] = expf((float)lc * t.lambda_thres / 255.0f - 2.5f);
    o[4] = decode_color(t.colors[l][px * 3 + 0], t.sigmoid_codec);
    o[5] = decode_color(t.colors[l][px * 3 + 1], t.sigmoid_codec);
    o[6] = decode_color(t.colors[l][px * 3 + 2], t.sigmoid_codec);
}

__global__ void texture_fetch_kernel(TexArgs t, const int64_t *texel, int64_t n, float *features)
{
    const int width = 3 + 7 * t.n_lobes + 1;
    for (int64_t i = (int64_t)blockIdx.x * blockDim.x + threadIdx.x; i < n; i += (int64_t)gridDim.x * blockDim.x) {
        const int64_t px = texel[i * 2] * t.size + texel[i * 2 + 1];
        float *f = features + i * width;
        const float a = (float)t.alpha[px] / 255.0f;
        f[0] = decode_color(t.diffuse[px * 3 + 0], t.sigmoid_codec);
        f[1] = decode_color(t.diffuse[px * 3 + 1], t.sigmoid_codec);
        f[2] = decode_color(t.diffuse[px * 3 + 2], t.sigmoid_codec);
#pragma unroll
        for (int l = 0; l < QF_MAX_LOBES; ++l) {
            if (l < t.n_lobes) {
                float o[7];
                decode_lobe(t, l, px, o);
#pragma unroll
                for (int k = 0; k < 7; ++k) f[3 + 7 * l + k] = o[k];
            }
        }
        f[width - 1] = -logf(fmaxf(1.0f - a, 1e-6f)) / 0.005f;
    }
}

__global__ void texture_shade_kernel(TexArgs t, const int64_t *texel, const float *dirs, int64_t n, float *rgb,
                                     float *sigma)
{
    for (int64_t i = (int64_t)blockIdx.x * blockDim.x + threadIdx.x; i < n; i += (int64_t)gridDim.x * blockDim.x) {
        const int64_t px = texel[i * 2] * t.size + texel[i * 2 + 1];
        const float dx = dirs[i * 3], dy = dirs[i * 3 + 1], dz = dirs[i * 3 + 2];
        float r = 0.0f, g = 0.0f, b = 0.0f;
#pragma unroll
        for (int l = 0; l < QF_MAX_LOBES; ++l) {
            if (l < t.n_lobes) {
                float x[7];
                decode_lobe(t, l, px, x);
                const float nrm = sqrtf((x[0] * x[0] + x[1] * x[1]) + x[2] * x[2]);
                const float dotp = ((x[0] / nrm) * dx + (x[1] / nrm) * dy) + (x[2] / nrm) * dz;
                const float e = expf(fabsf(x[3]) * (dotp - 1.0f));
                r += x[4] * e;
                g += x[5] * e;
                b += x[6] * e;
            }
        }
        rgb[i * 3 + 0] = 1.0f / (1.0f + expf(-(decode_color(t.diffuse[px * 3 + 0], t.sigmoid_codec) + r)));
        rgb[i * 3 + 1] = 1.0f / (1.0f + expf(-(decode_color(t.diffuse[px * 3 + 1], t.sigmoid_codec) + g)));
        rgb[i * 3 + 2] = 1.0f / (1.0f + expf(-(decode_color(t.diffuse[px * 3 + 2], t.sigmoid_codec) + b)));
        const float a = (float)t.alpha[px] / 255.0f;
        sigma[i] = -logf(fmaxf(1.0f - a, 1e-6f)) / 0.005f;
    }
}

int fill_tex_args(const qf_texture_set *tex, TexArgs *t)
{
    if (!tex || !tex->alpha || !tex->diffuse || tex->texture_size < 1) return QF_ERR_INVALID_ARGUMENT;
    if (tex->n_lobes < 1 || tex->n_lobes > QF_MAX_LOBES) return QF_ERR_UNSUPPORTED;
    t->alpha = tex->alpha;
    t->diffuse = tex->diffuse;
    for (int l = 0; l < QF_MAX_LOBES; ++l) {
        t->colors[l] = l < tex->n_lobes ? tex->colors[l] : nullptr;
        t->lam[l] = l < tex->n_lobes ? tex->lambda_axis[l] : nullptr;
        if (l < tex->n_lobes && (!t->colors[l] || !t->lam[l])) return QF_ERR_INVALID_ARGUMENT;
    }
    t->size = tex->texture_size;
    t->n_lobes = tex->n_lobes;
    t->sigmoid_codec = tex->sigmoid_codec;
    t->lambda_thres = tex->lambda_thres;
    return QF_OK;
}

}

#define QF_SIMPLE_LAUNCH(kernel, count, ...)                                                                  \
    hipLaunchKernelGGL(kernel, dim3(qf_grid_1d((count), 256)), dim3(256), 0, qf_stream(stream), __VA_ARGS__); \
    QF_LAUNCH_CHECK();

static int bvh_launch(const qf_bvh *bvh, const float *rays_o, const float *rays_d, int64_t n_rays, int32_t max_hits,
                      int32_t image_width, int32_t *hit_tri, float *hit_t, int32_t *hit_count, int only_overflowed,
                      uint64_t *keep_mask, int32_t *raw_count, void *stream, const int32_t *all_flag = nullptr)
{
    if (!bvh || n_rays < 0 || max_hits < 1 || max_hits > kMaxHits || image_width < 0) return QF_ERR_INVALID_ARGUMENT;
    if (bvh->n_tri >= (1 << 28)) return QF_ERR_UNSUPPORTED;
    if (n_rays == 0) return QF_OK;
    if (!rays_o || !rays_d || !hit_tri || !hit_t || !hit_count) return QF_ERR_INVALID_ARGUMENT;
    int height = 0, tiles_x = 0;
    int64_t n_blocks = qf_div_up(n_rays, kOctRays);
    if (image_width > 0) {
        if (n_rays % image_width) return QF_ERR_INVALID_ARGUMENT;
        height = (int)(n_rays / image_width);
        tiles_x = (image_width + 7) / 8;
        n_blocks = (int64_t)tiles_x * ((height + 3) / 4);
    }
    const bool sep = bvh->min_sep > 0.0f;
    const int stack_cap = (bvh->max_stack8 < 2 ? 2 : bvh->max_stack8) | 1;
    const int list_cap = (sep && only_overflowed) ? (max_hits + 8 < kMaxHits ? max_hits + 8 : kMaxHits) : max_hits;
    size_t lds = (size_t)kOctRays * ((size_t)list_cap * 8 * (sep ? 2 : 1) + (size_t)stack_cap * 4);
    const size_t tcol_offset = (lds + 3) / 4;
    if (only_overflowed && sep && keep_mask) lds = tcol_offset * 4 + (size_t)kTravThreads * max_hits * 4;
    if (lds > 160 * 1024 - 2048) return QF_ERR_UNSUPPORTED;
    TravArgs a;
    a.nodes = reinterpret_cast<const float4 *>(bvh->d_nodes8);
    a.tris = reinterpret_cast<const float4 *>(bvh->d_tris);
    a.rays_o = rays_o; a.rays_d = rays_d; a.n_rays = n_rays;
    a.root_is_valid = bvh->n_tri > 0 ? 1 : 0;
    a.max_hits = (int)max_hits; a.image_width = (int)image_width; a.image_height = height; a.tiles_x = tiles_x;
    a.stack_cap = stack_cap; a.list_cap = list_cap; a.min_sep = sep ? bvh->min_sep : 0.0f;
    a.hit_tri = hit_tri; a.hit_t = hit_t; a.hit_count = hit_count;
    a.keep_mask = (only_overflowed && sep) ? keep_mask : nullptr;
    a.raw_count = a.keep_mask ? raw_count : nullptr;
    a.tcol_offset = (int)tcol_offset;
    a.all_flag = only_overflowed ? all_flag : nullptr;
    if (only_overflowed) n_blocks = qf_div_up(n_rays, kTravThreads);
    int64_t per_xcd = qf_div_up(n_blocks, 8);
    a.stripe_blocks = 0;
    if (!only_overflowed) {
        a.stripe_blocks = image_width > 0 ? tiles_x * 2 : 256;
        if (n_blocks < (int64_t)a.stripe_blocks * (image_width > 0 ? 16 : 32)) a.stripe_blocks = 0;
    }
    if (a.stripe_blocks > 0) {
        const int64_t stripes = qf_div_up(n_blocks, a.stripe_blocks);
        per_xcd = qf_div_up(stripes, 8) * a.stripe_blocks;
    }
    if (per_xcd * 8 > 0x7fffffff) return QF_ERR_UNSUPPORTED;
    a.n_blocks = (int)n_blocks; a.blocks_per_xcd = (int)per_xcd;
    const bool ordered = bvh->depth_complexity >= 0.5f * (float)max_hits;
    const void *fn = only_overflowed ? reinterpret_cast<const void *>(bvh8_repair_kernel)
                                     : (ordered ? reinterpret_cast<const void *>(bvh8_traverse_kernel<true>)
                                                : reinterpret_cast<const void *>(bvh8_traverse_kernel<false>));
    if (lds > 48 * 1024) QF_HIP_TRY(hipFuncSetAttribute(fn, hipFuncAttributeMaxDynamicSharedMemorySize, (int)lds));
    if (only_overflowed)
        hipLaunchKernelGGL(bvh8_repair_kernel, dim3((unsigned)(per_xcd * 8)), dim3(kTravThreads), lds, qf_stream(stream), a);
    else if (ordered)
        hipLaunchKernelGGL(bvh8_traverse_kernel<true>, dim3((unsigned)(per_xcd * 8)), dim3(kTravThreads), lds, qf_stream(stream), a);
    else
        hipLaunchKernelGGL(bvh8_traverse_kernel<false>, dim3((unsigned)(per_xcd * 8)), dim3(kTravThreads), lds, qf_stream(stream), a);
    QF_LAUNCH_CHECK();
    return QF_OK;
}

static int filter_launch(int64_t n_rays, int32_t max_hits, float min_sep, int32_t *hit_tri, float *hit_t,
                         int32_t *hit_count, hipStream_t st)
{
    const int Kp = max_hits | 1;
    const size_t lds = (size_t)kFilterRays * Kp * 8;
    const int64_t blocks = qf_div_up(n_rays, kFilterRays);
    if (blocks > 0x7fffffff) return QF_ERR_UNSUPPORTED;
    hipLaunchKernelGGL(filter_hits_kernel, dim3((unsigned)blocks), dim3(kFilterRays), lds, st, n_rays, (int)max_hits, min_sep,
                       hit_tri, hit_t, hit_count);
    QF_LAUNCH_CHECK();
    return QF_OK;
}

extern "C" int qf_filter_hits(const qf_bvh *bvh, int64_t n_rays, int32_t max_hits, int32_t *hit_tri, float *hit_t,
                              int32_t *hit_count, void *stream)
{
    if (!bvh || n_rays < 0 || max_hits < 1 || max_hits > kMaxHits) return QF_ERR_INVALID_ARGUMENT;
    if (n_rays == 0 || !(bvh->min_sep > 0.0f)) return QF_OK;
    if (!hit_tri || !hit_t || !hit_count) return QF_ERR_INVALID_ARGUMENT;
    return filter_launch(n_rays, max_hits, bvh->min_sep, hit_tri, hit_t, hit_count, qf_stream(stream));
}

extern "C" int qf_bvh_intersect(const qf_bvh *bvh, const float *rays_o, const float *rays_d, int64_t n_rays,
                                int32_t max_hits, int32_t image_width, int32_t *hit_tri, float *hit_t,
                                int32_t *hit_count, void *stream)
{
    return bvh_launch(bvh, rays_o, rays_d, n_rays, max_hits, image_width, hit_tri, hit_t, hit_count, 0, nullptr, nullptr,
                      stream);
}

extern "C" int qf_bvh_repair_overflow(const qf_bvh *bvh, const float *rays_o, const float *rays_d, int64_t n_rays,
                                      int32_t max_hits, int32_t image_width, int32_t *hit_tri, float *hit_t,
                                      int32_t *hit_count, uint64_t *keep_mask, int32_t *raw_count,
                                      const int32_t *traverse_all_flag, void *stream)
{
    if ((keep_mask == nullptr) != (raw_count == nullptr)) return QF_ERR_INVALID_ARGUMENT;
    return bvh_launch(bvh, rays_o, rays_d, n_rays, max_hits, image_width, hit_tri, hit_t, hit_count, 1, keep_mask, raw_count,
                      stream, traverse_all_flag);
}

extern "C" int qf_pack_samples(const float *rays_o, const float *rays_d, int64_t n_rays, int32_t max_hits,
                               const int32_t *hit_tri, const float *hit_t, const int32_t *hit_count,
                               const int64_t *ray_offset, float *xyz, float *dirs, int64_t *index_ray, float *depth,
                               int64_t *index_tri, float *origins, const int32_t *inverse, float *xyz_c, float *dirs_c,
                               float *depth_c, const uint64_t *keep_mask, const int32_t *raw_count,
                               float min_separation, int32_t *close_flag, void *stream)
{
    if ((keep_mask == nullptr) != (raw_count == nullptr)) return QF_ERR_INVALID_ARGUMENT;
    if (n_rays < 0 || max_hits < 1 || max_hits > kMaxHits) return QF_ERR_INVALID_ARGUMENT;
    if (n_rays == 0) return QF_OK;
    if (!rays_o || !rays_d || !hit_tri || !hit_t || !hit_count || !ray_offset) return QF_ERR_INVALID_ARGUMENT;
    if (inverse && (!xyz_c || !dirs_c)) return QF_ERR_INVALID_ARGUMENT;
    if (!index_ray || !depth || !index_tri) return QF_ERR_INVALID_ARGUMENT;
    if ((xyz || dirs || origins) && (!xyz || !dirs || !origins)) return QF_ERR_INVALID_ARGUMENT;
    if (!xyz && !inverse) return QF_ERR_INVALID_ARGUMENT;
    const int Kp = max_hits | 1;
    const size_t lds = (size_t)kPackRays * Kp * 8 + (size_t)kPackRays * max_hits * 2 + 64;
    const int64_t blocks = qf_div_up(n_rays, kPackRays);
    if (blocks > 0x7fffffff) return QF_ERR_UNSUPPORTED;
    hipLaunchKernelGGL(pack_samples_kernel, dim3((unsigned)blocks), dim3(kPackRays), lds, qf_stream(stream), rays_o, rays_d,
                       n_rays, (int)max_hits, hit_tri, hit_t, hit_count, ray_offset, xyz, dirs, index_ray, depth, index_tri,
                       origins, inverse, xyz_c, dirs_c, depth_c, keep_mask, raw_count, min_separation, close_flag);
    QF_LAUNCH_CHECK();
    return QF_OK;
}

extern "C" int qf_pack_tiles(const float *rays_o, const float *rays_d, int32_t width, int32_t height, int32_t max_hits,
                             const int32_t *hit_tri, const float *hit_t, const int32_t *hit_count, const int64_t *tile_base,
                             const int64_t *total, float *xyz_c, float *dirs_c, float *depth_c, int32_t *tri_c,
                             const uint64_t *keep_mask, const int32_t *raw_count, float min_separation,
                             int32_t *final_count, int32_t *dropped, int64_t *host_out, int32_t dropped_is_zero,
                             void *stream)
{
    if ((keep_mask == nullptr) != (raw_count == nullptr)) return QF_ERR_INVALID_ARGUMENT;
    if (width < 1 || height < 1 || max_hits < 1 || max_hits > kMaxHits) return QF_ERR_INVALID_ARGUMENT;
    if (!rays_o || !rays_d || !hit_t || !hit_count || !tile_base || !total || !xyz_c || !dirs_c || !depth_c)
        return QF_ERR_INVALID_ARGUMENT;
    if (tri_c && !hit_tri) return QF_ERR_INVALID_ARGUMENT;
    const bool rule_here = !keep_mask && min_separation > 0.0f;
    if (rule_here && (!final_count || !dropped)) return QF_ERR_INVALID_ARGUMENT;
    if (host_out && !dropped) return QF_ERR_INVALID_ARGUMENT;
    hipStream_t st = qf_stream(stream);
    if (dropped && !host_out && !dropped_is_zero) QF_HIP_TRY(hipMemsetAsync(dropped, 0, sizeof(int32_t), st));
    const int tiles_x = (width + 7) / 8, tiles_y = (height + 7) / 8;
    const float sep = rule_here ? min_separation : 0.0f;
    if (tri_c) {
        hipLaunchKernelGGL(pack_tiles_kernel<true>, dim3((unsigned)(tiles_x * tiles_y)), dim3(64), (size_t)64 * (max_hits | 1) * 8, st,
                           rays_o, rays_d, (int)width, (int)height, tiles_x, tiles_x * tiles_y, (int)max_hits, hit_tri, hit_t,
                           hit_count, tile_base, total, xyz_c, dirs_c, depth_c, tri_c, keep_mask, raw_count, sep, final_count,
                           dropped);
    } else {
        hipLaunchKernelGGL(pack_tiles_kernel<false>, dim3((unsigned)(tiles_x * tiles_y)), dim3(64), (size_t)64 * (max_hits | 1) * 4, st,
                           rays_o, rays_d, (int)width, (int)height, tiles_x, tiles_x * tiles_y, (int)max_hits, hit_tri, hit_t,
                           hit_count, tile_base, total, xyz_c, dirs_c, depth_c, tri_c, keep_mask, raw_count, sep, final_count,
                           dropped);
    }
    if (host_out) hipLaunchKernelGGL(publish_dropped_kernel, dim3(1), dim3(1), 0, st, dropped, host_out);
    QF_LAUNCH_CHECK();
    return QF_OK;
}

extern "C" int qf_resort_by_depth(const int64_t *index_ray, const float *depth, int64_t n, int64_t *perm, void *stream)
{
    if (n < 0) return QF_ERR_INVALID_ARGUMENT;
    if (n == 0) return QF_OK;
    if (!index_ray || !depth || !perm) return QF_ERR_INVALID_ARGUMENT;
    QF_SIMPLE_LAUNCH(resort_kernel, n, index_ray, depth, n, perm);
    return QF_OK;
}

extern "C" int qf_resort_samples(const int64_t *index_ray, const float *depth, int64_t n, const float *points,
                                 const float *origins, const float *vectors, const int64_t *index_tri, int64_t *perm,
                                 float *out_points, float *out_depth, float *out_origins, float *out_vectors,
                                 int64_t *out_index_tri, uint8_t *boundary, const int32_t *inverse, float *out_points_c,
                                 float *out_vectors_c, void *stream)
{
    if (n < 0) return QF_ERR_INVALID_ARGUMENT;
    if (n == 0) return QF_OK;
    if (!index_ray || !depth || !points || !vectors || !out_points || !out_depth || !out_vectors ||
        (out_origins && !origins) || (out_index_tri && !index_tri) || (inverse && (!out_points_c || !out_vectors_c)))
        return QF_ERR_INVALID_ARGUMENT;
    const int64_t n_chunks = (n + RS_CHUNK - 1) / RS_CHUNK;
    hipLaunchKernelGGL(resort_samples_kernel, dim3((unsigned)(n_chunks < 65536 ? n_chunks : 65536)), dim3(RS_THREADS), 0,
                       qf_stream(stream), index_ray, depth, n, points, origins, vectors, index_tri, perm, out_points,
                       out_depth, out_origins, out_vectors, out_index_tri, boundary, inverse, out_points_c, out_vectors_c);
    QF_LAUNCH_CHECK();
    return QF_OK;
}

extern "C" int qf_texel_indices(const double *vertices, const int64_t *faces, const float *uv, const float *points,
                                const int64_t *index_tri, int64_t n, int32_t texture_size, int64_t *texel, void *stream)
{
    if (n < 0 || texture_size < 1) return QF_ERR_INVALID_ARGUMENT;
    if (n == 0) return QF_OK;
    if (!vertices || !faces || !uv || !points || !index_tri || !texel) return QF_ERR_INVALID_ARGUMENT;
    QF_SIMPLE_LAUNCH(texel_indices_kernel, n, vertices, faces, uv, points, index_tri, n, (int)texture_size, texel);
    return QF_OK;
}

extern "C" int qf_texel_records_pack(const double *vertices, const int64_t *faces, const float *uv, int64_t n_faces,
                                     void *records, void *stream)
{
    if (n_faces < 0) return QF_ERR_INVALID_ARGUMENT;
    if (n_faces == 0) return QF_OK;
    if (!vertices || !faces || !uv || !records) return QF_ERR_INVALID_ARGUMENT;
    QF_SIMPLE_LAUNCH(texel_records_kernel, n_faces, vertices, faces, uv, n_faces, static_cast<TexelRecord *>(records));
    return QF_OK;
}

extern "C" int qf_texel_indices_packed(const void *records, const float *points, const int64_t *index_tri, int64_t n,
                                       int32_t texture_size, int64_t *texel, void *stream)
{
    if (n < 0 || texture_size < 1) return QF_ERR_INVALID_ARGUMENT;
    if (n == 0) return QF_OK;
    if (!records || !points || !index_tri || !texel) return QF_ERR_INVALID_ARGUMENT;
    QF_SIMPLE_LAUNCH(texel_indices_packed_kernel, n, static_cast<const TexelRecord *>(records), points, index_tri, n,
                     (int)texture_size, texel);
    return QF_OK;
}

extern "C" int qf_texture_fetch(const qf_texture_set *tex, const int64_t *texel, int64_t n, float *features, void *stream)
{
    TexArgs t;
    int rc = fill_tex_args(tex, &t);
    if (rc != QF_OK) return rc;
    if (n < 0) return QF_ERR_INVALID_ARGUMENT;
    if (n == 0) return QF_OK;
    if (!texel || !features) return QF_ERR_INVALID_ARGUMENT;
    QF_SIMPLE_LAUNCH(texture_fetch_kernel, n, t, texel, n, features);
    return QF_OK;
}

extern "C" int qf_texture_shade(const qf_texture_set *tex, const int64_t *texel, const float *dirs, int64_t n,
                                float *rgb, float *sigma, void *stream)
{
    TexArgs t;
    int rc = fill_tex_args(tex, &t);
    if (rc != QF_OK) return rc;
    if (n < 0) return QF_ERR_INVALID_ARGUMENT;
    if (n == 0) return QF_OK;
    if (!texel || !dirs || !rgb || !sigma) return QF_ERR_INVALID_ARGUMENT;
    QF_SIMPLE_LAUNCH(texture_shade_kernel, n, t, texel, dirs, n, rgb, sigma);
    return QF_OK;
}

extern "C" int qf_texture_pack(const qf_texture_set *tex, uint8_t *records, void *stream)
{
    TexArgs t;
    int rc = fill_tex_args(tex, &t);
    if (rc != QF_OK) return rc;
    if (!records || 4 + 6 * t.n_lobes > kTexelRecord) return QF_ERR_INVALID_ARGUMENT;
    QF_SIMPLE_LAUNCH(texture_pack_kernel, (int64_t)t.size * t.size, t, records);
    return QF_OK;
}

extern "C" int qf_texture_shade_packed(const uint8_t *records, int32_t texture_size, int32_t n_lobes,
                                       int32_t sigmoid_codec, float lambda_thres, const int64_t *texel,
                                       const float *dirs, int64_t n, float *rgb, float *sigma, void *stream)
{
    if (!records || texture_size < 1 || n < 0) return QF_ERR_INVALID_ARGUMENT;
    if (n_lobes < 1 || n_lobes > QF_MAX_LOBES) return QF_ERR_UNSUPPORTED;
    if (n == 0) return QF_OK;
    if (!texel || !dirs || !rgb || !sigma) return QF_ERR_INVALID_ARGUMENT;
    QF_SIMPLE_LAUNCH((texture_shade_packed_kernel<false, int64_t>), n, records, (int)texture_size, (int)n_lobes,
                     (int)sigmoid_codec, lambda_thres, texel, dirs, n, rgb, sigma, (const TexelRecord *)nullptr,
                     (const float *)nullptr, (const int64_t *)nullptr, (const int64_t *)nullptr);
    return QF_OK;
}

extern "C" int qf_texture_shade_points(const uint8_t *records, int32_t texture_size, int32_t n_lobes, int32_t sigmoid_codec,
                                       float lambda_thres, const void *triangle_records, const float *points,
                                       const int64_t *index_tri, const int32_t *index_tri32, const float *dirs, int64_t n,
                                       const int64_t *n_device, float *rgb, float *sigma, void *stream)
{
    if (!records || !triangle_records || texture_size < 1 || n < 0) return QF_ERR_INVALID_ARGUMENT;
    if (n_lobes < 1 || n_lobes > QF_MAX_LOBES) return QF_ERR_UNSUPPORTED;
    if (n == 0) return QF_OK;
    if (!points || (!index_tri == !index_tri32) || !dirs || !rgb || !sigma) return QF_ERR_INVALID_ARGUMENT;
    const TexelRecord *tr = static_cast<const TexelRecord *>(triangle_records);
    if (index_tri32) {
        QF_SIMPLE_LAUNCH((texture_shade_packed_kernel<true, int32_t>), n, records, (int)texture_size, (int)n_lobes,
                         (int)sigmoid_codec, lambda_thres, (const int64_t *)nullptr, dirs, n, rgb, sigma, tr, points,
                         index_tri32, n_device);
    } else {
        QF_SIMPLE_LAUNCH((texture_shade_packed_kernel<true, int64_t>), n, records, (int)texture_size, (int)n_lobes,
                         (int)sigmoid_codec, lambda_thres, (const int64_t *)nullptr, dirs, n, rgb, sigma, tr, points,
                         index_tri, n_device);
    }
    return QF_OK;
}

static RasterCam make_raster_cam(const qf_camera *cam)
{
    RasterCam rc;
    const float *m = cam->c2w;
    rc.r00 = m[0]; rc.r01 = m[1]; rc.r02 = m[2]; rc.cx = m[3];
    rc.r10 = m[4]; rc.r11 = m[5]; rc.r12 = m[6]; rc.cy = m[7];
    rc.r20 = m[8]; rc.r21 = m[9]; rc.r22 = m[10]; rc.cz = m[11];
    rc.fx = cam->fx; rc.fy = cam->fy;
    rc.px0 = cam->cx - 0.5f;
    rc.py0 = cam->cy - 0.5f;
    rc.w = cam->width; rc.h = cam->height;
    return rc;
}

static int ensure_chunk_boxes(qf_bvh *bvh, hipStream_t st)
{
    const int64_t n_chunks = qf_div_up(bvh->n_tri, kCullChunk);
    if (n_chunks > 0x3fffffff) return QF_ERR_UNSUPPORTED;
    if (!bvh->d_chunk_box) {
        QF_HIP_TRY(hipMalloc((void **)&bvh->d_chunk_box, (size_t)n_chunks * 2 * sizeof(float4)));
        QF_HIP_TRY(hipMalloc((void **)&bvh->d_visible, (size_t)(n_chunks + 2) * sizeof(int32_t)));
        QF_HIP_TRY(hipMemsetAsync(bvh->d_visible, 0, 2 * sizeof(int32_t), st));
        bvh->chunk_dirty = true;
        bvh->cull_parity = 0;
    }
    if (bvh->chunk_dirty) {
        hipLaunchKernelGGL(chunk_boxes_kernel, dim3((unsigned)qf_div_up(n_chunks * 64, 256)), dim3(256), 0, st,
                           reinterpret_cast<const float4 *>(bvh->d_tris), bvh->n_tri, (int)n_chunks,
                           reinterpret_cast<float4 *>(bvh->d_chunk_box));
        QF_LAUNCH_CHECK();
        bvh->chunk_dirty = false;
    }
    return QF_OK;
}

static int raster_zero(int64_t n_rays, int32_t *hit_count, int32_t *overflow, int32_t *origin_flag, hipStream_t st)
{
    int64_t words = n_rays;
    bool ovf_done = false, flag_done = origin_flag == nullptr;
    if (overflow == hit_count + words) { ++words; ovf_done = true; }
    if (ovf_done && origin_flag == hit_count + words) { ++words; flag_done = true; }
    QF_HIP_TRY(hipMemsetAsync(hit_count, 0, (size_t)words * sizeof(int32_t), st));
    if (!ovf_done) QF_HIP_TRY(hipMemsetAsync(overflow, 0, sizeof(int32_t), st));
    if (!flag_done) QF_HIP_TRY(hipMemsetAsync(origin_flag, 0, sizeof(int32_t), st));
    return QF_OK;
}

static int raster_launch(qf_bvh *bvh, const qf_camera *cam, const float *rays_o, const float *rays_d, int64_t n_rays,
                         int capacity, bool wide, int32_t *hit_tri, float *hit_t, int32_t *hit_count, int32_t *overflow,
                         int32_t *origin_flag, bool cull, hipStream_t st, bool skip_ids = false)
{
    if (skip_ids) hit_tri = nullptr;
    const int rc_zero = raster_zero(n_rays, hit_count, overflow, origin_flag, st);
    if (rc_zero != QF_OK) return rc_zero;
    const RasterCam rc = make_raster_cam(cam);
    const uint32_t *o_bits = reinterpret_cast<const uint32_t *>(rays_o);
    if (bvh->n_tri > 0) {
        const int64_t pixels_per_tri = n_rays / bvh->n_tri;
        const int lanes = pixels_per_tri > 64 ? 16 : (pixels_per_tri > 8 ? 8 : 4);
        const int64_t threads = bvh->n_tri * lanes;
        const int64_t blocks = qf_div_up(threads, 256);
        if (blocks > 0x7fffffff) return QF_ERR_UNSUPPORTED;
        if (cull) {
            const int64_t n_chunks = qf_div_up(bvh->n_tri, kCullChunk);
            const int rc_boxes = ensure_chunk_boxes(bvh, st);
            if (rc_boxes != QF_OK) return rc_boxes;
            const float4 *tris4 = reinterpret_cast<const float4 *>(bvh->d_tris);
            float4 *boxes = reinterpret_cast<float4 *>(bvh->d_chunk_box);
            int32_t *counters = bvh->d_visible, *visible = bvh->d_visible + 2;
            const int parity = bvh->cull_parity;
            bvh->cull_parity ^= 1;
            hipLaunchKernelGGL(cull_chunks_kernel, dim3((unsigned)qf_div_up(n_chunks, 256)), dim3(256), 0, st, boxes,
                               (int)n_chunks, rc, visible, counters, parity, o_bits, rays_d, n_rays, origin_flag);
            QF_LAUNCH_CHECK();
            const int64_t items = n_chunks * (kCullChunk * lanes / 256);
            const int64_t cap = (int64_t)qf_cu_count_cached() * 8;
            const unsigned grid = (unsigned)(items < cap ? items : cap);
#define QF_RASTER_CULLED(L, WIDE)                                                                                      \
    hipLaunchKernelGGL((raster_culled_kernel<L, WIDE>), dim3(grid), dim3(256), 0, st, tris4, bvh->n_tri, rc, rays_o,  \
                       rays_d, capacity, hit_tri, hit_t, hit_count, overflow, visible, counters + parity, origin_flag)
            if (wide) {
                switch (lanes) {
                case 16: QF_RASTER_CULLED(16, true); break;
                case 8: QF_RASTER_CULLED(8, true); break;
                default: QF_RASTER_CULLED(4, true); break;
                }
            } else {
                switch (lanes) {
                case 16: QF_RASTER_CULLED(16, false); break;
                case 8: QF_RASTER_CULLED(8, false); break;
                default: QF_RASTER_CULLED(4, false); break;
                }
            }
#undef QF_RASTER_CULLED
            QF_LAUNCH_CHECK();
            return QF_OK;
        }
        if (origin_flag) {
            hipLaunchKernelGGL(camera_rays_check_kernel, dim3(qf_grid_1d(n_rays, 256)), dim3(256), 0, st, o_bits, rays_d, n_rays,
                               rc, origin_flag);
            QF_LAUNCH_CHECK();
        }
#define QF_RASTER_LAUNCH(L, WIDE)                                                                                     \
    hipLaunchKernelGGL((raster_kernel<L, WIDE>), dim3((unsigned)blocks), dim3(256), 0, st,                           \
                       reinterpret_cast<const float4 *>(bvh->d_tris), bvh->n_tri, rc, rays_o, rays_d, capacity,      \
                       hit_tri, hit_t, hit_count, overflow, origin_flag)
        if (wide) {
            switch (lanes) {
            case 16: QF_RASTER_LAUNCH(16, true); break;
            case 8: QF_RASTER_LAUNCH(8, true); break;
            default: QF_RASTER_LAUNCH(4, true); break;
            }
        } else {
            switch (lanes) {
            case 16: QF_RASTER_LAUNCH(16, false); break;
            case 8: QF_RASTER_LAUNCH(8, false); break;
            default: QF_RASTER_LAUNCH(4, false); break;
            }
        }
#undef QF_RASTER_LAUNCH
        QF_LAUNCH_CHECK();
    }
    return QF_OK;
}

static bool raster_args_ok(const qf_bvh *bvh, const qf_camera *cam, int64_t n_rays, int32_t max_hits)
{
    if (!bvh || !cam || n_rays < 0 || max_hits < 1 || max_hits > kMaxHits) return false;
    if (cam->width < 1 || cam->height < 1 || (int64_t)cam->width * cam->height != n_rays) return false;
    return cam->fx > 0.0f && cam->fy > 0.0f;
}

extern "C" int qf_raster_intersect(qf_bvh *bvh, const qf_camera *cam, const float *rays_o, const float *rays_d,
                                   int64_t n_rays, int32_t max_hits, int32_t *hit_tri, float *hit_t, int32_t *hit_count,
                                   int32_t *overflow, int32_t sort_lists, int32_t cull_chunks, int32_t *origin_flag,
                                   void *stream)
{
    if (!raster_args_ok(bvh, cam, n_rays, max_hits)) return QF_ERR_INVALID_ARGUMENT;
    if (!rays_o || !rays_d || !hit_tri || !hit_t || !hit_count || !overflow) return QF_ERR_INVALID_ARGUMENT;
    if (sort_lists < 0 || sort_lists > 2) return QF_ERR_INVALID_ARGUMENT;
    hipStream_t st = qf_stream(stream);
    const int rc = raster_launch(bvh, cam, rays_o, rays_d, n_rays, (int)max_hits, false, hit_tri, hit_t, hit_count, overflow,
                                 origin_flag, cull_chunks != 0, st, sort_lists == 2);
    if (rc != QF_OK) return rc;
    if (sort_lists == 1 && n_rays > 0) return filter_launch(n_rays, max_hits, bvh->min_sep, hit_tri, hit_t, hit_count, st);
    return QF_OK;
}

extern "C" int qf_raster_intersect_wide(qf_bvh *bvh, const qf_camera *cam, const float *rays_o, const float *rays_d,
                                        int64_t n_rays, int32_t max_hits, int32_t wide_hits, int32_t *wide_tri,
                                        float *wide_t, int32_t *hit_tri, float *hit_t, int32_t *hit_count,
                                        int32_t *overflow, int32_t cull_chunks, int32_t *origin_flag, void *stream)
{
    if (!raster_args_ok(bvh, cam, n_rays, max_hits)) return QF_ERR_INVALID_ARGUMENT;
    if (wide_hits < max_hits || wide_hits > 4096) return QF_ERR_INVALID_ARGUMENT;
    if (!rays_o || !rays_d || !wide_tri || !wide_t || !hit_tri || !hit_t || !hit_count || !overflow)
        return QF_ERR_INVALID_ARGUMENT;
    hipStream_t st = qf_stream(stream);
    const int rc = raster_launch(bvh, cam, rays_o, rays_d, n_rays, (int)wide_hits, true, wide_tri, wide_t, hit_count, overflow,
                                 origin_flag, cull_chunks != 0, st);
    if (rc != QF_OK) return rc;
    if (n_rays == 0) return QF_OK;
    const size_t lds = (size_t)select_capacity(max_hits, wide_hits, bvh->min_sep) * kSelectBlock * 2 * sizeof(float);
    hipLaunchKernelGGL(select_nearest_kernel<false>, dim3((unsigned)qf_div_up(n_rays, kSelectBlock)), dim3(kSelectBlock), lds, st,
                       n_rays, (int)wide_hits, (int)max_hits, bvh->min_sep, wide_tri, wide_t, (const uint64_t *)nullptr, hit_tri,
                       hit_t, hit_count);
    QF_LAUNCH_CHECK();
    return QF_OK;
}

namespace {
__global__ void slab_init_kernel(SlabCtl *ctl)
{
    ctl->dist_min_bits = 0x7f800000u;
    ctl->dist_max_bits = 0u;
    ctl->n_visible = 0;
    for (int j = 0; j < kMaxSlabs; ++j) ctl->slab_count[j] = 0;
}
}

extern "C" int qf_raster_intersect_slabs(qf_bvh *bvh, const qf_camera *cam, const float *rays_o, const float *rays_d,
                                         int64_t n_rays, int32_t max_hits, int32_t wide_hits, int32_t n_slabs,
                                         uint64_t *wide_keys, int32_t *hit_tri, float *hit_t, int32_t *hit_count,
                                         int32_t *overflow, int32_t *origin_flag, void *stream)
{
    if (!raster_args_ok(bvh, cam, n_rays, max_hits)) return QF_ERR_INVALID_ARGUMENT;
    if (n_slabs < 2 || n_slabs > kMaxSlabs) return QF_ERR_INVALID_ARGUMENT;
    const int sel_cap = select_capacity(max_hits, wide_hits, bvh->min_sep);
    if (wide_hits <= sel_cap + 1 || wide_hits > 4096) return QF_ERR_INVALID_ARGUMENT;
    if (!rays_o || !rays_d || !wide_keys || !hit_tri || !hit_t || !hit_count || !overflow) return QF_ERR_INVALID_ARGUMENT;
    hipStream_t st = qf_stream(stream);
    const int rc_zero = raster_zero(n_rays, hit_count, overflow, origin_flag, st);
    if (rc_zero != QF_OK) return rc_zero;
    if (n_rays == 0 || bvh->n_tri == 0) return QF_OK;
    const int rc_boxes = ensure_chunk_boxes(bvh, st);
    if (rc_boxes != QF_OK) return rc_boxes;
    const int64_t n_chunks = qf_div_up(bvh->n_tri, kCullChunk);
    if (!bvh->d_slab_range) {
        QF_HIP_TRY(hipMalloc((void **)&bvh->d_slab_range, (size_t)n_chunks * sizeof(float2)));
        QF_HIP_TRY(hipMalloc((void **)&bvh->d_slab_lists, (size_t)n_chunks * kMaxSlabs * sizeof(int32_t)));
        QF_HIP_TRY(hipMalloc((void **)&bvh->d_slab_ctl, sizeof(SlabCtl)));
    }
    const RasterCam rc = make_raster_cam(cam);
    const float4 *tris4 = reinterpret_cast<const float4 *>(bvh->d_tris);
    const float4 *boxes = reinterpret_cast<const float4 *>(bvh->d_chunk_box);
    int32_t *visible = bvh->d_visible + 2;
    float2 *range = reinterpret_cast<float2 *>(bvh->d_slab_range);
    SlabCtl *ctl = reinterpret_cast<SlabCtl *>(bvh->d_slab_ctl);
    if (origin_flag) {
        hipLaunchKernelGGL(camera_rays_check_kernel, dim3(qf_grid_1d(n_rays, 256)), dim3(256), 0, st,
                           reinterpret_cast<const uint32_t *>(rays_o), rays_d, n_rays, rc, origin_flag);
    }
    hipLaunchKernelGGL(slab_init_kernel, dim3(1), dim3(1), 0, st, ctl);
    hipLaunchKernelGGL(slab_cull_kernel, dim3((unsigned)qf_div_up(n_chunks, 256)), dim3(256), 0, st, boxes, (int)n_chunks, rc,
                       visible, range, ctl);
    hipLaunchKernelGGL(slab_assign_kernel, dim3((unsigned)qf_div_up(n_chunks, 256)), dim3(256), 0, st, visible, range, ctl,
                       (int)n_slabs, (int)n_chunks, bvh->d_slab_lists);
    QF_LAUNCH_CHECK();
    const int64_t pixels_per_tri = n_rays / bvh->n_tri;
    const int lanes = pixels_per_tri > 64 ? 16 : (pixels_per_tri > 8 ? 8 : 4);
    const int64_t items = n_chunks * (kCullChunk * lanes / 256);
    const int64_t cap = (int64_t)qf_cu_count_cached() * 8;
    const unsigned grid = (unsigned)(items < cap ? items : cap);
    const int stop_at = sel_cap + 1;
    if (bvh->slab_snapshot_rays < n_rays) {
        const int64_t grown = bvh->slab_snapshot_rays * 2 > n_rays ? bvh->slab_snapshot_rays * 2 : n_rays;
        if (bvh->d_slab_snapshot) (void)hipFree(bvh->d_slab_snapshot);
        bvh->d_slab_snapshot = nullptr;
        bvh->slab_snapshot_rays = 0;
        QF_HIP_TRY(hipMalloc((void **)&bvh->d_slab_snapshot, (size_t)grown * sizeof(float4)));
        bvh->slab_snapshot_rays = grown;
    }
    float4 *snapshot = reinterpret_cast<float4 *>(bvh->d_slab_snapshot);
    for (int j = 0; j < n_slabs; ++j) {
        if (j > 0) {
            hipLaunchKernelGGL(slab_ray_records_kernel, dim3(qf_grid_1d(n_rays, 256)), dim3(256), 0, st, rays_d, hit_count,
                               n_rays, snapshot);
            QF_LAUNCH_CHECK();
        }
        const int32_t *list = bvh->d_slab_lists + (int64_t)j * n_chunks;
#define QF_RASTER_SLAB(L)                                                                                              \
    hipLaunchKernelGGL((raster_slab_kernel<L>), dim3(grid), dim3(256), 0, st, tris4, bvh->n_tri, rc, rays_o, rays_d,    \
                       (int)wide_hits, wide_keys, hit_count, overflow, list, ctl, j, (int)n_slabs, stop_at,               \
                       j == 0 ? (const float4 *)nullptr : snapshot, origin_flag)
        switch (lanes) {
        case 16: QF_RASTER_SLAB(16); break;
        case 8: QF_RASTER_SLAB(8); break;
        default: QF_RASTER_SLAB(4); break;
        }
#undef QF_RASTER_SLAB
    }
    QF_LAUNCH_CHECK();
    const size_t lds = (size_t)sel_cap * kSelectBlock * 2 * sizeof(float);
    hipLaunchKernelGGL(select_nearest_kernel<true>, dim3((unsigned)qf_div_up(n_rays, kSelectBlock)), dim3(kSelectBlock), lds, st,
                       n_rays, (int)wide_hits, (int)max_hits, bvh->min_sep, (const int32_t *)nullptr, (const float *)nullptr,
                       wide_keys, hit_tri, hit_t, hit_count);
    QF_LAUNCH_CHECK();
    return QF_OK;
}

namespace {

struct MarchArgs {
    float lo[3], hi[3];
    int res[3];
    float near_plane, far_plane, step;
};

__device__ __forceinline__ bool march_range(const MarchArgs &m, const float *o, const float *d, float t_near_ray,
                                            float t_far_ray, float *t0, float *t1)
{
    float tn = -INFINITY, tf = INFINITY;
#pragma unroll
    for (int k = 0; k < 3; ++k) {
        const float inv = safe_inv(d[k]);
        const float a = (m.lo[k] - o[k]) * inv, b = (m.hi[k] - o[k]) * inv;
        tn = fmaxf(tn, fminf(a, b));
        tf = fminf(tf, fmaxf(a, b));
    }
    *t0 = fmaxf(tn, t_near_ray);
    *t1 = fminf(tf, t_far_ray);
    return tn <= tf && *t0 < *t1;
}

__device__ __forceinline__ bool march_occupied(const MarchArgs &m, const uint8_t *binaries, const float *o,
                                               const float *d, float tm)
{
    int c[3];
#pragma unroll
    for (int k = 0; k < 3; ++k) {
        const float p = o[k] + d[k] * tm;
        const float u = (p - m.lo[k]) / (m.hi[k] - m.lo[k]) * (float)m.res[k];
        const float f = floorf(u);
        if (!(f >= 0.0f && f < (float)m.res[k])) return false;
        c[k] = (int)f;
    }
    return binaries[((int64_t)c[0] * m.res[1] + c[1]) * m.res[2] + c[2]] != 0;
}

__global__ void grid_march_kernel(MarchArgs m, const uint8_t *binaries, const float *rays_o, const float *rays_d,
                                  const float *t_min, const float *t_max, int64_t n_rays, int32_t *count,
                                  const int64_t *offsets, float *t_starts, float *t_ends, int64_t *ray_indices)
{
    for (int64_t r = (int64_t)blockIdx.x * blockDim.x + threadIdx.x; r < n_rays; r += (int64_t)gridDim.x * blockDim.x) {
        const float o[3] = {rays_o[r * 3], rays_o[r * 3 + 1], rays_o[r * 3 + 2]};
        const float d[3] = {rays_d[r * 3], rays_d[r * 3 + 1], rays_d[r * 3 + 2]};
        const float near_r = t_min ? fmaxf(m.near_plane, t_min[r]) : m.near_plane;
        const float far_r = t_max ? fminf(m.far_plane, t_max[r]) : m.far_plane;
        float t0, t1;
        int n = 0;
        int64_t w = count ? 0 : offsets[r];
        if (march_range(m, o, d, near_r, far_r, &t0, &t1)) {
            for (int k = 0; k < (1 << 22); ++k) {
                const float ts = t0 + (float)k * m.step;
                const float te = t0 + (float)(k + 1) * m.step;
                const float tm = (ts + te) * 0.5f;
                if (!(tm < t1)) break;
                if (!march_occupied(m, binaries, o, d, tm)) continue;
                if (!count) { t_starts[w] = ts; t_ends[w] = te; ray_indices[w] = r; ++w; }
                ++n;
            }
        }
        if (count) count[r] = n;
    }
}

int fill_march_args(const float *aabb, const int32_t *res, float near_plane, float far_plane, float step, MarchArgs *m)
{
    if (!aabb || !res || !(step > 0.0f) || !(far_plane > near_plane)) return QF_ERR_INVALID_ARGUMENT;
    for (int k = 0; k < 3; ++k) {
        m->lo[k] = aabb[k];
        m->hi[k] = aabb[3 + k];
        m->res[k] = res[k];
        if (!(aabb[3 + k] > aabb[k]) || res[k] < 1) return QF_ERR_INVALID_ARGUMENT;
        if ((aabb[3 + k] - aabb[k]) / step > 1.0e7f) return QF_ERR_UNSUPPORTED;
    }
    m->near_plane = near_plane;
    m->far_plane = far_plane;
    m->step = step;
    return QF_OK;
}

}

extern "C" int qf_grid_march_count(const float *aabb, const int32_t *resolution, const uint8_t *binaries,
                                   const float *rays_o, const float *rays_d, const float *t_min, const float *t_max,
                                   int64_t n_rays, float near_plane, float far_plane, float step, int32_t *count,
                                   void *stream)
{
    MarchArgs m;
    int rc = fill_march_args(aabb, resolution, near_plane, far_plane, step, &m);
    if (rc != QF_OK) return rc;
    if (n_rays < 0) return QF_ERR_INVALID_ARGUMENT;
    if (n_rays == 0) return QF_OK;
    if (!binaries || !rays_o || !rays_d || !count) return QF_ERR_INVALID_ARGUMENT;
    hipLaunchKernelGGL(grid_march_kernel, dim3(qf_grid_1d(n_rays, 64, 64)), dim3(64), 0, qf_stream(stream), m, binaries,
                       rays_o, rays_d, t_min, t_max, n_rays, count, (const int64_t *)nullptr, (float *)nullptr,
                       (float *)nullptr, (int64_t *)nullptr);
    QF_LAUNCH_CHECK();
    return QF_OK;
}

extern "C" int qf_grid_march_write(const float *aabb, const int32_t *resolution, const uint8_t *binaries,
                                   const float *rays_o, const float *rays_d, const float *t_min, const float *t_max,
                                   int64_t n_rays, float near_plane, float far_plane, float step, const int64_t *offsets,
                                   float *t_starts, float *t_ends, int64_t *ray_indices, void *stream)
{
    MarchArgs m;
    int rc = fill_march_args(aabb, resolution, near_plane, far_plane, step, &m);
    if (rc != QF_OK) return rc;
    if (n_rays < 0) return QF_ERR_INVALID_ARGUMENT;
    if (n_rays == 0) return QF_OK;
    if (!binaries || !rays_o || !rays_d || !offsets) return QF_ERR_INVALID_ARGUMENT;
    hipLaunchKernelGGL(grid_march_kernel, dim3(qf_grid_1d(n_rays, 64, 64)), dim3(64), 0, qf_stream(stream), m, binaries,
                       rays_o, rays_d, t_min, t_max, n_rays, (int32_t *)nullptr, offsets, t_starts, t_ends, ray_indices);
    QF_LAUNCH_CHECK();
    return QF_OK;
}
```

### quadraturefields_amd/csrc/frame.cpp

```cpp
#include "qf_common.h"

extern "C" int qf_frame_render(qf_bvh *bvh, const qf_frame_job *job, void *stream)
{
    if (!bvh || !job || !job->camera) return QF_ERR_INVALID_ARGUMENT;
    const qf_frame_job &j = *job;
    const int32_t w = j.camera->width, h = j.camera->height;
    if (w < 1 || h < 1 || j.n_rays != (int64_t)w * h || j.max_hits < 1) return QF_ERR_INVALID_ARGUMENT;
    if (!j.rays_o || !j.rays_d || !j.hit_tri || !j.hit_t || !j.hit_count || !j.final_count || !j.tile_base || !j.total ||
        !j.dropped || !j.xyz_c || !j.dirs_c || !j.depth_c)
        return QF_ERR_INVALID_ARGUMENT;
    if (j.field_precision < QF_FIELD_FP32 || j.field_precision > QF_FIELD_FP16) return QF_ERR_INVALID_ARGUMENT;
    if (j.field) {
        const qf_field_desc &f = *j.field;
        if (!j.rgb_c || !j.sigma_c || !j.table || !j.base_w) return QF_ERR_INVALID_ARGUMENT;
        if (f.head == QF_HEAD_NGP) {
            if (!j.head_ngp_w) return QF_ERR_INVALID_ARGUMENT;
        } else if (f.head == QF_HEAD_SG) {
            if (!j.head_sg) return QF_ERR_INVALID_ARGUMENT;
            if (j.field_precision == QF_FIELD_FP32) {
                const qf_sg_head *s = static_cast<const qf_sg_head *>(j.head_sg);
                if (!s->w1 || !s->b1 || !s->w2 || !s->b2 || !s->wout || !s->bout) return QF_ERR_INVALID_ARGUMENT;
            } else {
                const qf_sg_head_bf16 *s = static_cast<const qf_sg_head_bf16 *>(j.head_sg);
                if (!s->w1 || !s->b1 || !s->w2 || !s->b2 || !s->wout || !s->bout) return QF_ERR_INVALID_ARGUMENT;
            }
            if (f.n_lobes < 1 || f.n_lobes > QF_MAX_LOBES) return QF_ERR_UNSUPPORTED;
        } else {
            return QF_ERR_INVALID_ARGUMENT;
        }
        for (int k = 0; k < 3; ++k)
            if (!(f.aabb[3 + k] > f.aabb[k])) return QF_ERR_INVALID_ARGUMENT;
        if (j.bg_mode < 0 || j.bg_mode > 3) return QF_ERR_INVALID_ARGUMENT;
        if (!j.out_packed && (!j.out_rgb || !j.out_alpha || !j.out_depth)) return QF_ERR_INVALID_ARGUMENT;
        if (j.bg_mode == QF_BG_CUSTOM && !j.bkgd) return QF_ERR_INVALID_ARGUMENT;
    }
    const int64_t cap = j.n_rays * (int64_t)j.max_hits;
    int32_t *overflow = j.hit_count + j.n_rays;
    int rc = qf_raster_intersect(bvh, j.camera, j.rays_o, j.rays_d, j.n_rays, j.max_hits, j.hit_tri, j.hit_t, j.hit_count,
                                 overflow, j.tri_c ? 0 : 2 , j.cull_chunks,
                                 overflow + 1, stream);
    if (rc != QF_OK) return rc;
    rc = qf_bvh_repair_overflow(bvh, j.rays_o, j.rays_d, j.n_rays, j.max_hits, w, j.hit_tri, j.hit_t, j.hit_count, nullptr,
                                nullptr, overflow + 1, stream);
    if (rc != QF_OK) return rc;
    rc = qf_tile_offsets(j.hit_count, j.max_hits, w, h, j.tile_base, j.total, overflow, overflow + 1, j.host_block, j.dropped,
                         stream);
    if (rc != QF_OK) return rc;
    rc = qf_pack_tiles(j.rays_o, j.rays_d, w, h, j.max_hits, j.hit_tri, j.hit_t, j.hit_count, j.tile_base, j.total, j.xyz_c,
                       j.dirs_c, j.depth_c, j.tri_c, nullptr, nullptr, j.min_separation, j.final_count, j.dropped, nullptr, 1,
                       stream);
    if (rc != QF_OK) return rc;
    if (!j.field) return QF_OK;
    if (j.field_precision == QF_FIELD_FP32) {
        rc = qf_field_forward(j.field, static_cast<const float *>(j.table), static_cast<const float *>(j.base_w),
                              static_cast<const float *>(j.head_ngp_w), static_cast<const qf_sg_head *>(j.head_sg),
                              j.xyz_c, j.dirs_c, cap, j.total, nullptr, j.rgb_c, j.sigma_c, nullptr, nullptr, nullptr,
                              stream);
    } else {
        auto fwd = j.field_precision == QF_FIELD_BF16 ? qf_field_forward_bf16 : qf_field_forward_f16;
        rc = fwd(j.field, static_cast<const uint16_t *>(j.table), static_cast<const uint16_t *>(j.base_w),
                 static_cast<const uint16_t *>(j.head_ngp_w), static_cast<const qf_sg_head_bf16 *>(j.head_sg), j.xyz_c,
                 j.dirs_c, cap, j.total, nullptr, j.rgb_c, j.sigma_c, nullptr, stream);
    }
    if (rc != QF_OK) return rc;
    return qf_composite_tiles(j.rgb_c, j.sigma_c, j.depth_c, j.delta_const, j.final_count, j.max_hits, j.tile_base, w, h,
                              j.bg_mode, j.bkgd, j.out_rgb, j.out_alpha, j.out_depth, nullptr, j.out_packed, stream);
}
```

### quadraturefields_amd/csrc/qf_common.h

```cpp
#pragma once
#include <hip/hip_runtime.h>
#include <stdint.h>

#include <atomic>

#include "qf_hip.h"

#define QF_HIP_TRY(expr)                       \
    do {                                       \
        hipError_t _e = (expr);                \
        if (_e != hipSuccess) {                \
            qf_set_last_hip_error((int)_e);    \
            return QF_ERR_HIP;                 \
        }                                      \
    } while (0)

#define QF_LAUNCH_CHECK()                      \
    do {                                       \
        hipError_t _e = hipGetLastError();     \
        if (_e != hipSuccess) {                \
            qf_set_last_hip_error((int)_e);    \
            return QF_ERR_HIP;                 \
        }                                      \
    } while (0)

extern "C" void qf_set_last_hip_error(int code);

static inline hipStream_t qf_stream(void *s) { return reinterpret_cast<hipStream_t>(s); }

int qf_cu_count_cached();

static inline int64_t qf_div_up(int64_t a, int64_t b) { return (a + b - 1) / b; }

static inline int qf_grid_1d(int64_t n, int block, int blocks_per_cu = 8)
{
    int64_t want = qf_div_up(n, block);
    int64_t cap = (int64_t)qf_cu_count_cached() * blocks_per_cu;
    if (want < 1) want = 1;
    return (int)(want < cap ? want : cap);
}

struct QfLdsAttr {
    std::atomic<bool> set[64];
};
static inline hipError_t qf_ensure_dynamic_lds(QfLdsAttr &a, const void *fn, size_t bytes)
{
    int dev = 0;
    hipError_t e = hipGetDevice(&dev);
    if (e != hipSuccess) return e;
    const bool tracked = dev >= 0 && dev < 64;
    if (tracked && a.set[dev].load(std::memory_order_acquire)) return hipSuccess;
    e = hipFuncSetAttribute(fn, hipFuncAttributeMaxDynamicSharedMemorySize, (int)bytes);
    if (e == hipSuccess && tracked) a.set[dev].store(true, std::memory_order_release);
    return e;
}

static inline int64_t qf_banded_tiles(int32_t width, int32_t height, int32_t band_rows)
{
    const int64_t tiles_x = (width + 7) / 8;
    if (band_rows <= 0 || band_rows >= height) return tiles_x * ((height + 7) / 8);
    const int64_t full = height / band_rows, rest = height - full * band_rows;
    return tiles_x * (full * ((band_rows + 7) / 8) + (rest + 7) / 8);
}

__device__ __forceinline__ int qf_tile_lane_ray(int tile, int lane, int w, int h, int tiles_x, int band_rows, int64_t *ray)
{
    const int px = (tile % tiles_x) * 8 + (lane & 7);
    int py;
    if (band_rows > 0 && band_rows < h) {
        const int per_band = tiles_x * ((band_rows + 7) / 8);
        const int band = tile / per_band, t = tile - band * per_band;
        const int local = (t / tiles_x) * 8 + (lane >> 3);
        if (local >= band_rows) return 0;
        py = band * band_rows + local;
    } else {
        py = (tile / tiles_x) * 8 + (lane >> 3);
    }
    if (px >= w || py >= h) return 0;
    *ray = (int64_t)py * w + px;
    return 1;
}
```

### quadraturefields_amd/csrc/scan.hip

```cpp
#include "qf_common.h"

namespace {

constexpr int kFoRays = 1024;
constexpr int kFoThreads = 256;

__device__ __forceinline__ int64_t clamped(const int32_t *hit_count, int64_t r, int64_t n, int32_t cap)
{
    if (r >= n) return 0;
    const int32_t c = hit_count[r];
    return c < 0 ? 0 : (c < cap ? c : cap);
}

__device__ __forceinline__ int64_t block_inclusive_scan(int64_t v, int64_t *s_wave, int64_t *total)
{
    const int lane = threadIdx.x & 63, wave = threadIdx.x >> 6;
#pragma unroll
    for (int off = 1; off < 64; off <<= 1) {
        const int64_t o = __shfl_up(v, off, 64);
        if (lane >= off) v += o;
    }
    if (lane == 63) s_wave[wave] = v;
    __syncthreads();
    int64_t base = 0, sum = 0;
    for (int w = 0; w < kFoThreads / 64; ++w) {
        if (w < wave) base += s_wave[w];
        sum += s_wave[w];
    }
    __syncthreads();
    *total = sum;
    return v + base;
}

__global__ __launch_bounds__(kFoThreads) void frame_partials_kernel(const int32_t *__restrict__ hit_count, int64_t n_rays,
                                                                    int32_t cap, int n_blocks, int w, int h, int tiles_x,
                                                                    int n_tiles, int64_t *__restrict__ partial,
                                                                    int64_t *__restrict__ tile_total, int band_rows)
{
    __shared__ int64_t s_wave[kFoThreads / 64];
    if ((int)blockIdx.x < n_blocks) {
        const int64_t r0 = (int64_t)blockIdx.x * kFoRays;
        int64_t v = 0;
#pragma unroll
        for (int k = 0; k < kFoRays / kFoThreads; ++k) v += clamped(hit_count, r0 + threadIdx.x + (int64_t)k * kFoThreads, n_rays, cap);
#pragma unroll
        for (int off = 32; off > 0; off >>= 1) v += __shfl_xor(v, off, 64);
        if ((threadIdx.x & 63) == 0) s_wave[threadIdx.x >> 6] = v;
        __syncthreads();
        if (threadIdx.x == 0) {
            int64_t s = 0;
            for (int q = 0; q < kFoThreads / 64; ++q) s += s_wave[q];
            partial[blockIdx.x] = s;
        }
        return;
    }
    const int tile = ((int)blockIdx.x - n_blocks) * (kFoThreads / 64) + (threadIdx.x >> 6), lane = threadIdx.x & 63;
    if (tile >= n_tiles) return;
    int64_t ray = 0;
    int64_t cnt = qf_tile_lane_ray(tile, lane, w, h, tiles_x, band_rows, &ray) ? clamped(hit_count, ray, n_rays, cap) : 0;
#pragma unroll
    for (int off = 32; off > 0; off >>= 1) cnt += __shfl_xor(cnt, off, 64);
    if (lane == 0) tile_total[tile] = cnt;
}

__device__ __forceinline__ void frame_scan_body(int64_t *partial, int n_blocks, int64_t *tile_total, int n_tiles,
                                                int64_t *grand_total, const int32_t *overflow_in, int64_t *host_out,
                                                int64_t *s_wave, const int32_t *ray_flag_in)
{
    for (int pass = 0; pass < 2; ++pass) {
        int64_t *a = pass == 0 ? partial : tile_total;
        const int m = pass == 0 ? n_blocks : n_tiles;
        if (!a) continue;
        const int per = (m + kFoThreads - 1) / kFoThreads;
        const int i0 = threadIdx.x * per, i1 = i0 + per < m ? i0 + per : m;
        int64_t sum = 0;
#pragma unroll 8
        for (int i = i0; i < i1; ++i) sum += a[i];
        int64_t total;
        int64_t run = block_inclusive_scan(sum, s_wave, &total) - sum;
#pragma unroll 8
        for (int i = i0; i < i1; ++i) {
            const int64_t v = a[i];
            a[i] = run;
            run += v;
        }
        if (threadIdx.x == 0 && (pass == 0 || !partial)) {
            *grand_total = total;
            if (host_out) {
                host_out[0] = total;
                host_out[1] = overflow_in ? (int64_t)*overflow_in : 0;
                host_out[3] = ray_flag_in ? (int64_t)*ray_flag_in : 0;
            }
        }
    }
}

__global__ __launch_bounds__(kFoThreads) void frame_scan_kernel(int64_t *partial, int n_blocks, int64_t *tile_total, int n_tiles,
                                                                int64_t *grand_total, const int32_t *overflow_in,
                                                                int64_t *host_out, int32_t *zero_word,
                                                                const int32_t *ray_flag_in)
{
    __shared__ int64_t s_wave[kFoThreads / 64];
    if (zero_word && threadIdx.x == 0) *zero_word = 0;
    frame_scan_body(partial, n_blocks, tile_total, n_tiles, grand_total, overflow_in, host_out, s_wave, ray_flag_in);
}

__global__ __launch_bounds__(kFoThreads) void frame_ray_offsets_kernel(const int32_t *__restrict__ hit_count, int64_t n_rays,
                                                                       int32_t cap, const int64_t *__restrict__ partial,
                                                                       int64_t *__restrict__ ray_offset)
{
    __shared__ int64_t s_wave[kFoThreads / 64];
    const int64_t r0 = (int64_t)blockIdx.x * kFoRays + (int64_t)threadIdx.x * (kFoRays / kFoThreads);
    int64_t c[kFoRays / kFoThreads], v = 0;
#pragma unroll
    for (int k = 0; k < kFoRays / kFoThreads; ++k) { c[k] = clamped(hit_count, r0 + k, n_rays, cap); v += c[k]; }
    int64_t total;
    int64_t run = partial[blockIdx.x] + block_inclusive_scan(v, s_wave, &total) - v;
#pragma unroll
    for (int k = 0; k < kFoRays / kFoThreads; ++k) {
        if (r0 + k < n_rays) ray_offset[r0 + k] = run;
        run += c[k];
    }
}

}

extern "C" int64_t qf_banded_tile_count(int32_t width, int32_t height, int32_t band_rows)
{
    if (width < 1 || height < 1 || band_rows < 0) return -1;
    return qf_banded_tiles(width, height, band_rows);
}

extern "C" int64_t qf_frame_offsets_temp_bytes(int64_t n_rays)
{
    if (n_rays < 0) return -1;
    return (qf_div_up(n_rays, kFoRays) + 1) * (int64_t)sizeof(int64_t);
}

extern "C" int qf_frame_offsets(const int32_t *hit_count, int64_t n_rays, int32_t max_hits, int32_t width, int32_t height,
                                int64_t *ray_offset, int64_t *tile_base, void *temp, int64_t temp_bytes,
                                const int32_t *overflow_in, const int32_t *ray_flag_in, int64_t *host_out, int32_t band_rows,
                                void *stream)
{
    if (n_rays < 0 || n_rays >= 0x7fffffff || max_hits < 1 || width < 0 || height < 0 || band_rows < 0)
        return QF_ERR_INVALID_ARGUMENT;
    if (!ray_offset || !temp || (n_rays > 0 && !hit_count)) return QF_ERR_INVALID_ARGUMENT;
    if (temp_bytes < qf_frame_offsets_temp_bytes(n_rays)) return QF_ERR_INVALID_ARGUMENT;
    const bool tiles = tile_base != nullptr;
    if (tiles && (width < 1 || height < 1 || (int64_t)width * height != n_rays)) return QF_ERR_INVALID_ARGUMENT;
    hipStream_t st = qf_stream(stream);
    const int n_blocks = (int)qf_div_up(n_rays, kFoRays);
    const int tiles_x = tiles ? (width + 7) / 8 : 0;
    const int n_tiles = tiles ? (int)qf_banded_tiles(width, height, band_rows) : 0;
    int64_t *partial = reinterpret_cast<int64_t *>(temp);
    const int tile_blocks = (int)qf_div_up(n_tiles, kFoThreads / 64);
    if (n_blocks + tile_blocks > 0) {
        hipLaunchKernelGGL(frame_partials_kernel, dim3((unsigned)(n_blocks + tile_blocks)), dim3(kFoThreads), 0, st, hit_count,
                           n_rays, max_hits, n_blocks, (int)width, (int)height, tiles_x, n_tiles, partial, tile_base,
                           (int)band_rows);
        QF_LAUNCH_CHECK();
    }
    hipLaunchKernelGGL(frame_scan_kernel, dim3(1), dim3(kFoThreads), 0, st, partial, n_blocks, tile_base, n_tiles,
                       ray_offset + n_rays, overflow_in, host_out, (int32_t *)nullptr, ray_flag_in);
    QF_LAUNCH_CHECK();
    if (n_blocks > 0) {
        hipLaunchKernelGGL(frame_ray_offsets_kernel, dim3((unsigned)n_blocks), dim3(kFoThreads), 0, st, hit_count, n_rays,
                           max_hits, partial, ray_offset);
        QF_LAUNCH_CHECK();
    }
    return QF_OK;
}

extern "C" int qf_tile_offsets(const int32_t *hit_count, int32_t max_hits, int32_t width, int32_t height,
                               int64_t *tile_base, int64_t *total, const int32_t *overflow_in, const int32_t *ray_flag_in,
                               int64_t *host_out, int32_t *zero_word, void *stream)
{
    if (max_hits < 1 || width < 1 || height < 1 || !hit_count || !tile_base || !total) return QF_ERR_INVALID_ARGUMENT;
    const int64_t n_rays = (int64_t)width * height;
    if (n_rays >= 0x7fffffff) return QF_ERR_INVALID_ARGUMENT;
    hipStream_t st = qf_stream(stream);
    const int tiles_x = (width + 7) / 8;
    const int n_tiles = tiles_x * ((height + 7) / 8);
    const int tile_blocks = (int)qf_div_up(n_tiles, kFoThreads / 64);
    hipLaunchKernelGGL(frame_partials_kernel, dim3((unsigned)tile_blocks), dim3(kFoThreads), 0, st, hit_count, n_rays, max_hits,
                       0, (int)width, (int)height, tiles_x, n_tiles, (int64_t *)nullptr, tile_base, 0);
    hipLaunchKernelGGL(frame_scan_kernel, dim3(1), dim3(kFoThreads), 0, st, (int64_t *)nullptr, 0, tile_base, n_tiles, total,
                       overflow_in, host_out, zero_word, ray_flag_in);
    QF_LAUNCH_CHECK();
    return QF_OK;
}

extern "C" int64_t qf_sample_offsets_temp_bytes(int64_t n_rays)
{
    const int64_t b = qf_frame_offsets_temp_bytes(n_rays);
    return b < 0 ? b : (b < 16 ? 16 : b);
}

extern "C" int qf_sample_offsets(const int32_t *hit_count, int64_t n_rays, int32_t max_hits, int64_t *ray_offset,
                                 void *temp, int64_t temp_bytes, void *stream)
{
    if (temp_bytes < qf_sample_offsets_temp_bytes(n_rays)) return QF_ERR_INVALID_ARGUMENT;
    return qf_frame_offsets(hit_count, n_rays, max_hits, 0, 0, ray_offset, nullptr, temp, temp_bytes, nullptr, nullptr,
                            nullptr, 0, stream);
}
```

Baseline: 399.9 million.

## Store per-ray hit lists in 8x8 tile-major interleaved layout

Adds a tile-ordered layout for hit_t/hit_tri/hit_count. Each 8x8 pixel tile's hits are stored contiguously with slot-major interleaving across the tile's pixels. Raster, BVH overflow repair, tile offset scan and tile packing all gain tiled variants, and the frame pipeline switches to them. The aim is coalesced reads in pack_tiles and tighter locality for raster atomics and writes. The cost is extra index arithmetic, strided per-ray writes during traversal, and a scalar strided load path in load_sort_row.

```diff
diff --git a/quadraturefields_amd/csrc/exact.hip b/quadraturefields_amd/csrc/exact.hip
--- a/quadraturefields_amd/csrc/exact.hip
+++ b/quadraturefields_amd/csrc/exact.hip
@@ -182,6 +182,7 @@
     int32_t *raw_count;
     int tcol_offset;
     const int32_t *all_flag;
+    int tile_order;
 };
 
 extern __shared__ uint64_t trav_lds[];
@@ -212,8 +213,8 @@
     return mask;
 }
 
-template <bool kOrdered>
-__device__ __forceinline__ void oct_traverse_ray(const TravArgs &ta, int64_t ray, int j, int q, int oct_base)
+template <bool kOrdered, bool kTiled = false>
+__device__ __forceinline__ void oct_traverse_ray(const TravArgs &ta, int64_t at, int j, int q, int oct_base)
 {
     const int K = ta.max_hits;
     const int Kc = ta.list_cap;
@@ -230,12 +231,22 @@
     int32_t *hit_tri = ta.hit_tri, *hit_count = ta.hit_count;
     uint64_t *keep_mask = ta.keep_mask;
     int32_t *raw_count = ta.raw_count;
+    int64_t ray = at, list_at = at * K;
+    int step = 1;
+    if (kTiled) {
+        int x, y;
+        qf_tile_pixel(at, ta.image_width, ta.image_height, &x, &y);
+        const QfTilePos tp = qf_tile_pos(x, y, ta.image_width, ta.image_height);
+        ray = (int64_t)y * ta.image_width + x;
+        list_at = tp.start * K + tp.local;
+        step = tp.size;
+    }
     const float ox = rays_o[ray * 3], oy = rays_o[ray * 3 + 1], oz = rays_o[ray * 3 + 2];
     const float dx = rays_d[ray * 3], dy = rays_d[ray * 3 + 1], dz = rays_d[ray * 3 + 2];
     const float ix = safe_inv(dx), iy = safe_inv(dy), iz = safe_inv(dz);
     const float nx = -(ox * ix), ny = -(oy * iy), nz = -(oz * iz);
-    float *my_t = hit_t + ray * K;
-    int32_t *my_tri = hit_tri + ray * K;
+    float *my_t = hit_t + list_at;
+    int32_t *my_tri = hit_tri + list_at;
 
     OctList list;
     list.keys = keys; list.K = Kc; list.j = j;
@@ -339,8 +350,8 @@
                 const uint64_t k = keys[e];
                 int rank = 0;
                 for (int i = 0; i < count; ++i) rank += keys[i] < k ? 1 : 0;
-                my_t[rank] = key_t(k);
-                my_tri[rank] = key_id(k);
+                my_t[rank * step] = key_t(k);
+                my_tri[rank * step] = key_id(k);
             }
             kept = count;
             break;
@@ -356,7 +367,7 @@
             const uint64_t k = sorted[i];
             const float t = key_t(k);
             if (kept == 0 || t > last_t + min_sep) {
-                if (j == 0) { my_t[kept] = t; my_tri[kept] = key_id(k); }
+                if (j == 0) { my_t[kept * step] = t; my_tri[kept * step] = key_id(k); }
                 ++kept;
                 last_t = t;
             }
@@ -367,10 +378,10 @@
         t_accept = last_t + min_sep;
         oct_lds_sync();
     }
-    for (int i = kept + j; i < K; i += 8) { my_t[i] = INFINITY; my_tri[i] = -1; }
+    for (int i = kept + j; i < K; i += 8) { my_t[i * step] = INFINITY; my_tri[i * step] = -1; }
     if (j == 0) {
-        hit_count[ray] = kept;
-        if (keep_mask) { keep_mask[ray] = kept >= 64 ? ~0ull : ((1ull << kept) - 1ull); raw_count[ray] = kept; }
+        hit_count[at] = kept;
+        if (!kTiled && keep_mask) { keep_mask[ray] = kept >= 64 ? ~0ull : ((1ull << kept) - 1ull); raw_count[ray] = kept; }
     }
 }
 
@@ -457,7 +468,8 @@
         const int entry = s_list[e];
         const int64_t ray = ray0 + (entry & 0xffff);
         if ((entry >> 16) == 2) {
-            oct_traverse_ray<true>(a, ray, j, q, oct_base);
+            if (a.tile_order) oct_traverse_ray<true, true>(a, ray, j, q, oct_base);
+            else oct_traverse_ray<true>(a, ray, j, q, oct_base);
         } else {
             const int c = a.hit_count[ray];
             int kept;
@@ -538,7 +550,7 @@
     return true;
 }
 
-template <int kRasterLanes, bool kWide, bool kSlab = false>
+template <int kRasterLanes, bool kWide, bool kSlab = false, bool kTiled = false>
 __device__ __forceinline__ void raster_triangle(const float4 *__restrict__ tris, int64_t tri_i, int sub, const RasterCam &cam,
                                                 const float *__restrict__ rays_o, const float *__restrict__ rays_d,
                                                 int max_hits, int32_t *__restrict__ hit_tri, float *__restrict__ hit_t,
@@ -586,9 +598,16 @@
             else atomicAdd(overflow, 1);
             continue;
         }
-        const int slot = atomicAdd(&hit_count[ray], 1);
+        int64_t at_count = ray, at_list = ray * max_hits, list_step = 1;
+        if (kTiled) {
+            const QfTilePos tp = qf_tile_pos(cx_, cy_, cam.w, cam.h);
+            at_count = tp.start + tp.local;
+            at_list = tp.start * max_hits + tp.local;
+            list_step = tp.size;
+        }
+        const int slot = atomicAdd(&hit_count[at_count], 1);
         if (slot < max_hits) {
-            const int64_t at = kWide ? (int64_t)slot * ((int64_t)cam.w * cam.h) + ray : ray * max_hits + slot;
+            const int64_t at = kWide ? (int64_t)slot * ((int64_t)cam.w * cam.h) + ray : at_list + slot * list_step;
             hit_t[at] = t;
             if (hit_tri) hit_tri[at] = id;
         } else {
@@ -597,7 +616,7 @@
     }
 }
 
-template <int kRasterLanes, bool kWide>
+template <int kRasterLanes, bool kWide, bool kTiled>
 __global__ __launch_bounds__(256) void raster_kernel(const float4 *__restrict__ tris, int64_t n_tri, RasterCam cam,
                                                      const float *__restrict__ rays_o, const float *__restrict__ rays_d,
                                                      int max_hits, int32_t *__restrict__ hit_tri, float *__restrict__ hit_t,
@@ -610,8 +629,8 @@
     if (tri_i >= n_tri) return;
     if (ray_flag && *ray_flag) return;
     const bool cam_origin = ray_flag != nullptr;
-    raster_triangle<kRasterLanes, kWide>(tris, tri_i, sub, cam, rays_o, rays_d, max_hits, hit_tri, hit_t, hit_count, overflow,
-                                         cam_origin);
+    raster_triangle<kRasterLanes, kWide, false, kTiled>(tris, tri_i, sub, cam, rays_o, rays_d, max_hits, hit_tri, hit_t,
+                                                         hit_count, overflow, cam_origin);
 }
 
 constexpr float kRayPixelTol = 0.02f;
@@ -706,7 +725,7 @@
     if (keep) visible[atomicAdd(&counters[parity], 1)] = chunk;
 }
 
-template <int kRasterLanes, bool kWide>
+template <int kRasterLanes, bool kWide, bool kTiled>
 __global__ __launch_bounds__(256) void raster_culled_kernel(const float4 *__restrict__ tris, int64_t n_tri, RasterCam cam,
                                                             const float *__restrict__ rays_o, const float *__restrict__ rays_d,
                                                             int max_hits, int32_t *__restrict__ hit_tri, float *__restrict__ hit_t,
@@ -724,8 +743,8 @@
         const int chunk = visible[item / kBlocksPerChunk];
         const int64_t tri_i = (int64_t)chunk * kCullChunk + (item % kBlocksPerChunk) * kTrisPerBlock + threadIdx.x / kRasterLanes;
         if (tri_i < n_tri)
-            raster_triangle<kRasterLanes, kWide>(tris, tri_i, sub, cam, rays_o, rays_d, max_hits, hit_tri, hit_t, hit_count, overflow,
-                                                 cam_origin);
+            raster_triangle<kRasterLanes, kWide, false, kTiled>(tris, tri_i, sub, cam, rays_o, rays_d, max_hits, hit_tri, hit_t,
+                                                                 hit_count, overflow, cam_origin);
     }
 }
 
@@ -1049,7 +1068,7 @@
 
 template <int kN, bool kTri>
 __device__ __forceinline__ void load_sort_row(const float *__restrict__ g_t, const int32_t *__restrict__ g_i, int K,
-                                              int cnt, int deepest, float *row_t, int32_t *row_i)
+                                              int cnt, int deepest, float *row_t, int32_t *row_i, int step = 1)
 {
     float t[kN];
     int32_t id[kN];
@@ -1057,7 +1076,14 @@
     for (int j = 0; j < kN / 4; ++j) {
         f32x4u v = {INFINITY, INFINITY, INFINITY, INFINITY};
         i32x4u w = {-1, -1, -1, -1};
-        if (4 * j < deepest) {
+        if (4 * j < deepest && step != 1) {
+#pragma unroll
+            for (int e = 0; e < 4; ++e)
+                if (4 * j + e < K) {
+                    v[e] = g_t[(int64_t)(4 * j + e) * step];
+                    if (kTri) w[e] = g_i[(int64_t)(4 * j + e) * step];
+                }
+        } else if (4 * j < deepest) {
             if (4 * j + 3 < K) {
                 v = *reinterpret_cast<const f32x4u *>(g_t + 4 * j);
                 if (kTri) w = *reinterpret_cast<const i32x4u *>(g_i + 4 * j);
@@ -1278,7 +1304,8 @@
     const int32_t *__restrict__ hit_tri, const float *__restrict__ hit_t, const int32_t *__restrict__ hit_count,
     const int64_t *__restrict__ tile_base, const int64_t *__restrict__ total, float *__restrict__ xyz_c,
     float *__restrict__ dirs_c, float *__restrict__ depth_c, int32_t *__restrict__ tri_c, const uint64_t *__restrict__ keep_mask,
-    const int32_t *__restrict__ raw_count, float min_sep, int32_t *__restrict__ final_count, int32_t *__restrict__ dropped)
+    const int32_t *__restrict__ raw_count, float min_sep, int32_t *__restrict__ final_count, int32_t *__restrict__ dropped,
+    int tile_order)
 {
     extern __shared__ __attribute__((aligned(16))) unsigned char smem[];
     const int K = max_hits, Kp = max_hits | 1;
@@ -1290,9 +1317,13 @@
     const int px = px0 + (lane & 7), py = py0 + (lane >> 3);
     const bool inside = px < w && py < h;
     const int64_t ray = inside ? (int64_t)py * w + px : 0;
+    const int64_t start = (int64_t)py0 * w + (int64_t)px0 * rows;
+    const int size = cols * rows, local = inside ? (lane >> 3) * cols + (lane & 7) : 0;
+    const int64_t list = tile_order ? start * K + local : ray * K;
+    const int step = tile_order ? size : 1;
     int cnt = 0;
     if (inside) {
-        cnt = keep_mask ? raw_count[ray] : hit_count[ray];
+        cnt = keep_mask ? raw_count[ray] : hit_count[tile_order ? start + local : ray];
         if (cnt > K) cnt = K;
     }
     int deepest = cnt;
@@ -1311,8 +1342,16 @@
     const float dx = rays_d[ray * 3], dy = rays_d[ray * 3 + 1], dz = rays_d[ray * 3 + 2];
     int64_t base = tile_base[tile];
     if (K <= 32) {
-        if (deepest <= 16) load_sort_row<16, kTri>(hit_t + ray * K, hit_tri + ray * K, K, cnt, deepest, row_t, row_i);
-        else load_sort_row<32, kTri>(hit_t + ray * K, hit_tri + ray * K, K, cnt, deepest, row_t, row_i);
+        if (deepest <= 16) load_sort_row<16, kTri>(hit_t + list, hit_tri + list, K, cnt, deepest, row_t, row_i, step);
+        else load_sort_row<32, kTri>(hit_t + list, hit_tri + list, K, cnt, deepest, row_t, row_i, step);
+    } else if (tile_order) {
+        for (int i = lane; i < size * deepest; i += 64) {
+            const int k = i / size, l = i - k * size;
+            const int at = ((l / cols) * 8 + l % cols) * Kp + k;
+            s_t[at] = hit_t[start * K + i];
+            if (kTri) s_tri[at] = hit_tri[start * K + i];
+        }
+        __syncthreads();
     } else {
         for (int yy = 0; yy < rows; ++yy) {
             const int64_t row_ray0 = (int64_t)(py0 + yy) * w + px0;
@@ -1883,9 +1922,11 @@
 
 static int bvh_launch(const qf_bvh *bvh, const float *rays_o, const float *rays_d, int64_t n_rays, int32_t max_hits,
                       int32_t image_width, int32_t *hit_tri, float *hit_t, int32_t *hit_count, int only_overflowed,
-                      uint64_t *keep_mask, int32_t *raw_count, void *stream, const int32_t *all_flag = nullptr)
+                      uint64_t *keep_mask, int32_t *raw_count, void *stream, const int32_t *all_flag = nullptr,
+                      bool tile_order = false)
 {
     if (!bvh || n_rays < 0 || max_hits < 1 || max_hits > kMaxHits || image_width < 0) return QF_ERR_INVALID_ARGUMENT;
+    if (tile_order && (!only_overflowed || keep_mask || image_width == 0)) return QF_ERR_INVALID_ARGUMENT;
     if (bvh->n_tri >= (1 << 28)) return QF_ERR_UNSUPPORTED;
     if (n_rays == 0) return QF_OK;
     if (!rays_o || !rays_d || !hit_tri || !hit_t || !hit_count) return QF_ERR_INVALID_ARGUMENT;
@@ -1916,6 +1957,7 @@
     a.raw_count = a.keep_mask ? raw_count : nullptr;
     a.tcol_offset = (int)tcol_offset;
     a.all_flag = only_overflowed ? all_flag : nullptr;
+    a.tile_order = tile_order ? 1 : 0;
     if (only_overflowed) n_blocks = qf_div_up(n_rays, kTravThreads);
     int64_t per_xcd = qf_div_up(n_blocks, 8);
     a.stripe_blocks = 0;
@@ -1982,6 +2024,14 @@
     if ((keep_mask == nullptr) != (raw_count == nullptr)) return QF_ERR_INVALID_ARGUMENT;
     return bvh_launch(bvh, rays_o, rays_d, n_rays, max_hits, image_width, hit_tri, hit_t, hit_count, 1, keep_mask, raw_count,
                       stream, traverse_all_flag);
+}
+
+int qf_bvh_repair_overflow_tiled(const qf_bvh *bvh, const float *rays_o, const float *rays_d, int64_t n_rays,
+                                 int32_t max_hits, int32_t image_width, int32_t *hit_tri, float *hit_t, int32_t *hit_count,
+                                 const int32_t *traverse_all_flag, void *stream)
+{
+    return bvh_launch(bvh, rays_o, rays_d, n_rays, max_hits, image_width, hit_tri, hit_t, hit_count, 1, nullptr, nullptr,
+                      stream, traverse_all_flag, true);
 }
 
 extern "C" int qf_pack_samples(const float *rays_o, const float *rays_d, int64_t n_rays, int32_t max_hits,
@@ -2010,13 +2060,14 @@
     return QF_OK;
 }
 
-extern "C" int qf_pack_tiles(const float *rays_o, const float *rays_d, int32_t width, int32_t height, int32_t max_hits,
+static int pack_tiles_launch(const float *rays_o, const float *rays_d, int32_t width, int32_t height, int32_t max_hits,
                              const int32_t *hit_tri, const float *hit_t, const int32_t *hit_count, const int64_t *tile_base,
                              const int64_t *total, float *xyz_c, float *dirs_c, float *depth_c, int32_t *tri_c,
                              const uint64_t *keep_mask, const int32_t *raw_count, float min_separation,
                              int32_t *final_count, int32_t *dropped, int64_t *host_out, int32_t dropped_is_zero,
-                             void *stream)
-{
+                             void *stream, bool tile_order)
+{
+    if (tile_order && keep_mask) return QF_ERR_INVALID_ARGUMENT;
     if ((keep_mask == nullptr) != (raw_count == nullptr)) return QF_ERR_INVALID_ARGUMENT;
     if (width < 1 || height < 1 || max_hits < 1 || max_hits > kMaxHits) return QF_ERR_INVALID_ARGUMENT;
     if (!rays_o || !rays_d || !hit_t || !hit_count || !tile_base || !total || !xyz_c || !dirs_c || !depth_c)
@@ -2033,16 +2084,38 @@
         hipLaunchKernelGGL(pack_tiles_kernel<true>, dim3((unsigned)(tiles_x * tiles_y)), dim3(64), (size_t)64 * (max_hits | 1) * 8, st,
                            rays_o, rays_d, (int)width, (int)height, tiles_x, tiles_x * tiles_y, (int)max_hits, hit_tri, hit_t,
                            hit_count, tile_base, total, xyz_c, dirs_c, depth_c, tri_c, keep_mask, raw_count, sep, final_count,
-                           dropped);
+                           dropped, tile_order ? 1 : 0);
     } else {
         hipLaunchKernelGGL(pack_tiles_kernel<false>, dim3((unsigned)(tiles_x * tiles_y)), dim3(64), (size_t)64 * (max_hits | 1) * 4, st,
                            rays_o, rays_d, (int)width, (int)height, tiles_x, tiles_x * tiles_y, (int)max_hits, hit_tri, hit_t,
                            hit_count, tile_base, total, xyz_c, dirs_c, depth_c, tri_c, keep_mask, raw_count, sep, final_count,
-                           dropped);
+                           dropped, tile_order ? 1 : 0);
     }
     if (host_out) hipLaunchKernelGGL(publish_dropped_kernel, dim3(1), dim3(1), 0, st, dropped, host_out);
     QF_LAUNCH_CHECK();
     return QF_OK;
+}
+
+extern "C" int qf_pack_tiles(const float *rays_o, const float *rays_d, int32_t width, int32_t height, int32_t max_hits,
+                             const int32_t *hit_tri, const float *hit_t, const int32_t *hit_count, const int64_t *tile_base,
+                             const int64_t *total, float *xyz_c, float *dirs_c, float *depth_c, int32_t *tri_c,
+                             const uint64_t *keep_mask, const int32_t *raw_count, float min_separation,
+                             int32_t *final_count, int32_t *dropped, int64_t *host_out, int32_t dropped_is_zero,
+                             void *stream)
+{
+    return pack_tiles_launch(rays_o, rays_d, width, height, max_hits, hit_tri, hit_t, hit_count, tile_base, total, xyz_c,
+                             dirs_c, depth_c, tri_c, keep_mask, raw_count, min_separation, final_count, dropped, host_out,
+                             dropped_is_zero, stream, false);
+}
+
+int qf_pack_tiles_tiled(const float *rays_o, const float *rays_d, int32_t width, int32_t height, int32_t max_hits,
+                        const int32_t *hit_tri, const float *hit_t, const int32_t *hit_count, const int64_t *tile_base,
+                        const int64_t *total, float *xyz_c, float *dirs_c, float *depth_c, int32_t *tri_c,
+                        float min_separation, int32_t *final_count, int32_t *dropped, int32_t dropped_is_zero, void *stream)
+{
+    return pack_tiles_launch(rays_o, rays_d, width, height, max_hits, hit_tri, hit_t, hit_count, tile_base, total, xyz_c,
+                             dirs_c, depth_c, tri_c, nullptr, nullptr, min_separation, final_count, dropped, nullptr,
+                             dropped_is_zero, stream, true);
 }
 
 extern "C" int qf_resort_by_depth(const int64_t *index_ray, const float *depth, int64_t n, int64_t *perm, void *stream)
@@ -2224,8 +2297,9 @@
 
 static int raster_launch(qf_bvh *bvh, const qf_camera *cam, const float *rays_o, const float *rays_d, int64_t n_rays,
                          int capacity, bool wide, int32_t *hit_tri, float *hit_t, int32_t *hit_count, int32_t *overflow,
-                         int32_t *origin_flag, bool cull, hipStream_t st, bool skip_ids = false)
-{
+                         int32_t *origin_flag, bool cull, hipStream_t st, bool skip_ids = false, bool tiled = false)
+{
+    if (tiled && wide) return QF_ERR_UNSUPPORTED;
     if (skip_ids) hit_tri = nullptr;
     const int rc_zero = raster_zero(n_rays, hit_count, overflow, origin_flag, st);
     if (rc_zero != QF_OK) return rc_zero;
@@ -2252,20 +2326,27 @@
             const int64_t items = n_chunks * (kCullChunk * lanes / 256);
             const int64_t cap = (int64_t)qf_cu_count_cached() * 8;
             const unsigned grid = (unsigned)(items < cap ? items : cap);
-#define QF_RASTER_CULLED(L, WIDE)                                                                                      \
-    hipLaunchKernelGGL((raster_culled_kernel<L, WIDE>), dim3(grid), dim3(256), 0, st, tris4, bvh->n_tri, rc, rays_o,  \
-                       rays_d, capacity, hit_tri, hit_t, hit_count, overflow, visible, counters + parity, origin_flag)
+#define QF_RASTER_CULLED(L, WIDE, TILED)                                                                               \
+    hipLaunchKernelGGL((raster_culled_kernel<L, WIDE, TILED>), dim3(grid), dim3(256), 0, st, tris4, bvh->n_tri, rc,      \
+                       rays_o, rays_d, capacity, hit_tri, hit_t, hit_count, overflow, visible, counters + parity,        \
+                       origin_flag)
             if (wide) {
                 switch (lanes) {
-                case 16: QF_RASTER_CULLED(16, true); break;
-                case 8: QF_RASTER_CULLED(8, true); break;
-                default: QF_RASTER_CULLED(4, true); break;
+                case 16: QF_RASTER_CULLED(16, true, false); break;
+                case 8: QF_RASTER_CULLED(8, true, false); break;
+                default: QF_RASTER_CULLED(4, true, false); break;
+                }
+            } else if (tiled) {
+                switch (lanes) {
+                case 16: QF_RASTER_CULLED(16, false, true); break;
+                case 8: QF_RASTER_CULLED(8, false, true); break;
+                default: QF_RASTER_CULLED(4, false, true); break;
                 }
             } else {
                 switch (lanes) {
-                case 16: QF_RASTER_CULLED(16, false); break;
-                case 8: QF_RASTER_CULLED(8, false); break;
-                default: QF_RASTER_CULLED(4, false); break;
+                case 16: QF_RASTER_CULLED(16, false, false); break;
+                case 8: QF_RASTER_CULLED(8, false, false); break;
+                default: QF_RASTER_CULLED(4, false, false); break;
                 }
             }
 #undef QF_RASTER_CULLED
@@ -2277,21 +2358,27 @@
                                rc, origin_flag);
             QF_LAUNCH_CHECK();
         }
-#define QF_RASTER_LAUNCH(L, WIDE)                                                                                     \
-    hipLaunchKernelGGL((raster_kernel<L, WIDE>), dim3((unsigned)blocks), dim3(256), 0, st,                           \
+#define QF_RASTER_LAUNCH(L, WIDE, TILED)                                                                              \
+    hipLaunchKernelGGL((raster_kernel<L, WIDE, TILED>), dim3((unsigned)blocks), dim3(256), 0, st,                    \
                        reinterpret_cast<const float4 *>(bvh->d_tris), bvh->n_tri, rc, rays_o, rays_d, capacity,      \
                        hit_tri, hit_t, hit_count, overflow, origin_flag)
         if (wide) {
             switch (lanes) {
-            case 16: QF_RASTER_LAUNCH(16, true); break;
-            case 8: QF_RASTER_LAUNCH(8, true); break;
-            default: QF_RASTER_LAUNCH(4, true); break;
+            case 16: QF_RASTER_LAUNCH(16, true, false); break;
+            case 8: QF_RASTER_LAUNCH(8, true, false); break;
+            default: QF_RASTER_LAUNCH(4, true, false); break;
+            }
+        } else if (tiled) {
+            switch (lanes) {
+            case 16: QF_RASTER_LAUNCH(16, false, true); break;
+            case 8: QF_RASTER_LAUNCH(8, false, true); break;
+            default: QF_RASTER_LAUNCH(4, false, true); break;
             }
         } else {
             switch (lanes) {
-            case 16: QF_RASTER_LAUNCH(16, false); break;
-            case 8: QF_RASTER_LAUNCH(8, false); break;
-            default: QF_RASTER_LAUNCH(4, false); break;
+            case 16: QF_RASTER_LAUNCH(16, false, false); break;
+            case 8: QF_RASTER_LAUNCH(8, false, false); break;
+            default: QF_RASTER_LAUNCH(4, false, false); break;
             }
         }
 #undef QF_RASTER_LAUNCH
@@ -2321,6 +2408,16 @@
     if (rc != QF_OK) return rc;
     if (sort_lists == 1 && n_rays > 0) return filter_launch(n_rays, max_hits, bvh->min_sep, hit_tri, hit_t, hit_count, st);
     return QF_OK;
+}
+
+int qf_raster_intersect_tiled(qf_bvh *bvh, const qf_camera *cam, const float *rays_o, const float *rays_d, int64_t n_rays,
+                              int32_t max_hits, int32_t *hit_tri, float *hit_t, int32_t *hit_count, int32_t *overflow,
+                              int32_t skip_ids, int32_t cull_chunks, int32_t *origin_flag, void *stream)
+{
+    if (!raster_args_ok(bvh, cam, n_rays, max_hits)) return QF_ERR_INVALID_ARGUMENT;
+    if (!rays_o || !rays_d || !hit_tri || !hit_t || !hit_count || !overflow) return QF_ERR_INVALID_ARGUMENT;
+    return raster_launch(bvh, cam, rays_o, rays_d, n_rays, (int)max_hits, false, hit_tri, hit_t, hit_count, overflow,
+                         origin_flag, cull_chunks != 0, qf_stream(stream), skip_ids != 0, true);
 }
 
 extern "C" int qf_raster_intersect_wide(qf_bvh *bvh, const qf_camera *cam, const float *rays_o, const float *rays_d,
diff --git a/quadraturefields_amd/csrc/frame.cpp b/quadraturefields_amd/csrc/frame.cpp
--- a/quadraturefields_amd/csrc/frame.cpp
+++ b/quadraturefields_amd/csrc/frame.cpp
@@ -36,19 +36,18 @@
     }
     const int64_t cap = j.n_rays * (int64_t)j.max_hits;
     int32_t *overflow = j.hit_count + j.n_rays;
-    int rc = qf_raster_intersect(bvh, j.camera, j.rays_o, j.rays_d, j.n_rays, j.max_hits, j.hit_tri, j.hit_t, j.hit_count,
-                                 overflow, j.tri_c ? 0 : 2 , j.cull_chunks,
-                                 overflow + 1, stream);
+    int rc = qf_raster_intersect_tiled(bvh, j.camera, j.rays_o, j.rays_d, j.n_rays, j.max_hits, j.hit_tri, j.hit_t,
+                                       j.hit_count, overflow, j.tri_c ? 0 : 1 ,
+                                       j.cull_chunks, overflow + 1, stream);
     if (rc != QF_OK) return rc;
-    rc = qf_bvh_repair_overflow(bvh, j.rays_o, j.rays_d, j.n_rays, j.max_hits, w, j.hit_tri, j.hit_t, j.hit_count, nullptr,
-                                nullptr, overflow + 1, stream);
+    rc = qf_bvh_repair_overflow_tiled(bvh, j.rays_o, j.rays_d, j.n_rays, j.max_hits, w, j.hit_tri, j.hit_t, j.hit_count,
+                                      overflow + 1, stream);
     if (rc != QF_OK) return rc;
-    rc = qf_tile_offsets(j.hit_count, j.max_hits, w, h, j.tile_base, j.total, overflow, overflow + 1, j.host_block, j.dropped,
-                         stream);
+    rc = qf_tile_offsets_tiled(j.hit_count, j.max_hits, w, h, j.tile_base, j.total, overflow, overflow + 1, j.host_block,
+                               j.dropped, stream);
     if (rc != QF_OK) return rc;
-    rc = qf_pack_tiles(j.rays_o, j.rays_d, w, h, j.max_hits, j.hit_tri, j.hit_t, j.hit_count, j.tile_base, j.total, j.xyz_c,
-                       j.dirs_c, j.depth_c, j.tri_c, nullptr, nullptr, j.min_separation, j.final_count, j.dropped, nullptr, 1,
-                       stream);
+    rc = qf_pack_tiles_tiled(j.rays_o, j.rays_d, w, h, j.max_hits, j.hit_tri, j.hit_t, j.hit_count, j.tile_base, j.total,
+                             j.xyz_c, j.dirs_c, j.depth_c, j.tri_c, j.min_separation, j.final_count, j.dropped, 1, stream);
     if (rc != QF_OK) return rc;
     if (!j.field) return QF_OK;
     if (j.field_precision == QF_FIELD_FP32) {
diff --git a/quadraturefields_amd/csrc/qf_common.h b/quadraturefields_amd/csrc/qf_common.h
--- a/quadraturefields_amd/csrc/qf_common.h
+++ b/quadraturefields_amd/csrc/qf_common.h
@@ -80,3 +80,46 @@
     *ray = (int64_t)py * w + px;
     return 1;
 }
+
+struct QfTilePos {
+    int64_t start;
+    int size;
+    int local;
+};
+
+__device__ __forceinline__ QfTilePos qf_tile_pos(int x, int y, int w, int h)
+{
+    const int tx = x >> 3, ty = y >> 3;
+    const int cols = w - 8 * tx < 8 ? w - 8 * tx : 8, rows = h - 8 * ty < 8 ? h - 8 * ty : 8;
+    QfTilePos p;
+    p.start = (int64_t)ty * 8 * w + (int64_t)tx * 8 * rows;
+    p.size = cols * rows;
+    p.local = (y & 7) * cols + (x & 7);
+    return p;
+}
+
+__device__ __forceinline__ void qf_tile_pixel(int64_t i, int w, int h, int *x, int *y)
+{
+    const int ty = (int)(i / (8 * (int64_t)w));
+    const int rows = h - 8 * ty < 8 ? h - 8 * ty : 8;
+    const int64_t in_row = i - (int64_t)ty * 8 * w;
+    const int tx = (int)(in_row / (8 * rows));
+    const int cols = w - 8 * tx < 8 ? w - 8 * tx : 8;
+    const int local = (int)(in_row - (int64_t)tx * 8 * rows);
+    *y = 8 * ty + local / cols;
+    *x = 8 * tx + local % cols;
+}
+
+int qf_raster_intersect_tiled(qf_bvh *bvh, const qf_camera *cam, const float *rays_o, const float *rays_d, int64_t n_rays,
+                              int32_t max_hits, int32_t *hit_tri, float *hit_t, int32_t *hit_count, int32_t *overflow,
+                              int32_t skip_ids, int32_t cull_chunks, int32_t *origin_flag, void *stream);
+int qf_bvh_repair_overflow_tiled(const qf_bvh *bvh, const float *rays_o, const float *rays_d, int64_t n_rays,
+                                 int32_t max_hits, int32_t image_width, int32_t *hit_tri, float *hit_t, int32_t *hit_count,
+                                 const int32_t *traverse_all_flag, void *stream);
+int qf_tile_offsets_tiled(const int32_t *hit_count, int32_t max_hits, int32_t width, int32_t height, int64_t *tile_base,
+                          int64_t *total, const int32_t *overflow_in, const int32_t *ray_flag_in, int64_t *host_out,
+                          int32_t *zero_word, void *stream);
+int qf_pack_tiles_tiled(const float *rays_o, const float *rays_d, int32_t width, int32_t height, int32_t max_hits,
+                        const int32_t *hit_tri, const float *hit_t, const int32_t *hit_count, const int64_t *tile_base,
+                        const int64_t *total, float *xyz_c, float *dirs_c, float *depth_c, int32_t *tri_c,
+                        float min_separation, int32_t *final_count, int32_t *dropped, int32_t dropped_is_zero, void *stream);
diff --git a/quadraturefields_amd/csrc/scan.hip b/quadraturefields_amd/csrc/scan.hip
--- a/quadraturefields_amd/csrc/scan.hip
+++ b/quadraturefields_amd/csrc/scan.hip
@@ -35,7 +35,8 @@
 __global__ __launch_bounds__(kFoThreads) void frame_partials_kernel(const int32_t *__restrict__ hit_count, int64_t n_rays,
                                                                     int32_t cap, int n_blocks, int w, int h, int tiles_x,
                                                                     int n_tiles, int64_t *__restrict__ partial,
-                                                                    int64_t *__restrict__ tile_total, int band_rows)
+                                                                    int64_t *__restrict__ tile_total, int band_rows,
+                                                                    int tile_order)
 {
     __shared__ int64_t s_wave[kFoThreads / 64];
     if ((int)blockIdx.x < n_blocks) {
@@ -57,7 +58,14 @@
     const int tile = ((int)blockIdx.x - n_blocks) * (kFoThreads / 64) + (threadIdx.x >> 6), lane = threadIdx.x & 63;
     if (tile >= n_tiles) return;
     int64_t ray = 0;
-    int64_t cnt = qf_tile_lane_ray(tile, lane, w, h, tiles_x, band_rows, &ray) ? clamped(hit_count, ray, n_rays, cap) : 0;
+    int64_t cnt;
+    if (tile_order) {
+        const int px0 = (tile % tiles_x) * 8, py0 = (tile / tiles_x) * 8;
+        const int cols = w - px0 < 8 ? w - px0 : 8, rows = h - py0 < 8 ? h - py0 : 8;
+        cnt = lane < cols * rows ? clamped(hit_count, (int64_t)py0 * w + (int64_t)px0 * rows + lane, n_rays, cap) : 0;
+    } else {
+        cnt = qf_tile_lane_ray(tile, lane, w, h, tiles_x, band_rows, &ray) ? clamped(hit_count, ray, n_rays, cap) : 0;
+    }
 #pragma unroll
     for (int off = 32; off > 0; off >>= 1) cnt += __shfl_xor(cnt, off, 64);
     if (lane == 0) tile_total[tile] = cnt;
@@ -157,7 +165,7 @@
     if (n_blocks + tile_blocks > 0) {
         hipLaunchKernelGGL(frame_partials_kernel, dim3((unsigned)(n_blocks + tile_blocks)), dim3(kFoThreads), 0, st, hit_count,
                            n_rays, max_hits, n_blocks, (int)width, (int)height, tiles_x, n_tiles, partial, tile_base,
-                           (int)band_rows);
+                           (int)band_rows, 0);
         QF_LAUNCH_CHECK();
     }
     hipLaunchKernelGGL(frame_scan_kernel, dim3(1), dim3(kFoThreads), 0, st, partial, n_blocks, tile_base, n_tiles,
@@ -171,9 +179,9 @@
     return QF_OK;
 }
 
-extern "C" int qf_tile_offsets(const int32_t *hit_count, int32_t max_hits, int32_t width, int32_t height,
+static int tile_offsets_launch(const int32_t *hit_count, int32_t max_hits, int32_t width, int32_t height,
                                int64_t *tile_base, int64_t *total, const int32_t *overflow_in, const int32_t *ray_flag_in,
-                               int64_t *host_out, int32_t *zero_word, void *stream)
+                               int64_t *host_out, int32_t *zero_word, void *stream, bool tile_order)
 {
     if (max_hits < 1 || width < 1 || height < 1 || !hit_count || !tile_base || !total) return QF_ERR_INVALID_ARGUMENT;
     const int64_t n_rays = (int64_t)width * height;
@@ -183,13 +191,29 @@
     const int n_tiles = tiles_x * ((height + 7) / 8);
     const int tile_blocks = (int)qf_div_up(n_tiles, kFoThreads / 64);
     hipLaunchKernelGGL(frame_partials_kernel, dim3((unsigned)tile_blocks), dim3(kFoThreads), 0, st, hit_count, n_rays, max_hits,
-                       0, (int)width, (int)height, tiles_x, n_tiles, (int64_t *)nullptr, tile_base, 0);
+                       0, (int)width, (int)height, tiles_x, n_tiles, (int64_t *)nullptr, tile_base, 0, tile_order ? 1 : 0);
     hipLaunchKernelGGL(frame_scan_kernel, dim3(1), dim3(kFoThreads), 0, st, (int64_t *)nullptr, 0, tile_base, n_tiles, total,
                        overflow_in, host_out, zero_word, ray_flag_in);
     QF_LAUNCH_CHECK();
     return QF_OK;
 }
 
+extern "C" int qf_tile_offsets(const int32_t *hit_count, int32_t max_hits, int32_t width, int32_t height,
+                               int64_t *tile_base, int64_t *total, const int32_t *overflow_in, const int32_t *ray_flag_in,
+                               int64_t *host_out, int32_t *zero_word, void *stream)
+{
+    return tile_offsets_launch(hit_count, max_hits, width, height, tile_base, total, overflow_in, ray_flag_in, host_out,
+                               zero_word, stream, false);
+}
+
+int qf_tile_offsets_tiled(const int32_t *hit_count, int32_t max_hits, int32_t width, int32_t height, int64_t *tile_base,
+                          int64_t *total, const int32_t *overflow_in, const int32_t *ray_flag_in, int64_t *host_out,
+                          int32_t *zero_word, void *stream)
+{
+    return tile_offsets_launch(hit_count, max_hits, width, height, tile_base, total, overflow_in, ray_flag_in, host_out,
+                               zero_word, stream, true);
+}
+
 extern "C" int64_t qf_sample_offsets_temp_bytes(int64_t n_rays)
 {
     const int64_t b = qf_frame_offsets_temp_bytes(n_rays);
```

After: 400.9 million (median of 6 runs). No clear change (+0.2%).
